# lRomul/sensorium

Hardware: AMD Instinct MI355X
Metric: training clips/sec/GPU (DwiseNeuro fwd+bwd, B=32 T=32 36x64) at 1/2/4/8 GPUs (higher is better)
Workload: dtype bf16

## Files before the change

include/dwn.h:

```cpp
#ifndef DWN_H_
#define DWN_H_
#include <stddef.h>
#include <stdint.h>

#ifdef __cplusplus
extern "C" {
#endif

#define DWN_ABI_VERSION 7
#define DWN_F32 0
#define DWN_BF16 1
#define DWN_F32_AUTO 0
#define DWN_F32_NATIVE 1
#define DWN_F32_SPLIT3 2
#define DWN_BN_EVAL 0
#define DWN_BN_TRAIN 1
#define DWN_BN_FROZEN 2
#define DWN_NREP 32

#define DWN_LD_PLAIN 0
#define DWN_LD_PE 1
#define DWN_LD_BNACT 2
#define DWN_LD_AFFINE2 3
#define DWN_LD_DY3 4
// ... 85 lines not shown
    void* dh1;
    float* dw;
    int planes, Hin, Win, Hout, Wout, C, stride, ks;
    double* stats;
    int rows_band;
    int impl;
    const void* a0; long long a0_ld; const void* w1; int Cin;
} dwn_dw_spatial_bwd_args;

typedef struct dwn_dw_temporal_fwd_args {
    dwn_load_desc in;
    const float* w;
    void* out;
    int B, T, HW, C, kt;
    double* stats;
    const float* z_scale; const float* z_shift; long long* pooled;
} dwn_dw_temporal_fwd_args;

typedef struct dwn_dw_temporal_bwd_args {
    dwn_load_desc dy; int dy_kind;
    dwn_load_desc y2;
    const float* w;
    void* dh2;
    float* dw;
    int B, T, HW, C, kt;
    double* stats;
} dwn_dw_temporal_bwd_args;

typedef struct dwn_bn {
    const float* gamma; const float* beta;
    float* running_mean; float* running_var; long long* num_batches_tracked;
    float* coef;
    float* dgamma; float* dbeta;
} dwn_bn;

typedef struct dwn_stem_args {
    int dtype, training, B, Cin, C0; long long S;
    float eps, momentum;
    const float* x;
    const float* w;
    dwn_bn bn;
    const float *pe_t, *pe_h, *pe_w;
    int T, H, W;
    void* y0;
    void* out;
    const void* dout;
    float* dw;
    void* ws; size_t ws_bytes;
    double* xmom;
} dwn_stem_args;

typedef struct dwn_stem_input_grad_args {
    int dtype, training, B, Cin, C0; long long S;
    const float* w;
    const float* coef;
    const void* dout;
    float* dx;
} dwn_stem_input_grad_args;

typedef struct dwn_block_args {
    int dtype, training;
    int B, T, Hin, Win, Hout, Wout, Cin, Cmid, Cout, stride, ks, kt, se_r;
    float eps, momentum;
    const void* x; void* out;
    void *y1, *y2, *y3, *y4;
    void* z3;
    int x_has_pe;
    void* a0;
    const float *pe_t, *pe_h, *pe_w;
    const float *out_pe_t, *out_pe_h, *out_pe_w;
    const float *w_pw, *w_dws, *w_dwt, *w_pwl, *se_wr, *se_br, *se_we, *se_be;
    dwn_bn bn1, bn2, bn3, bn4, bnsc;
    const float* drop_scale;
    const int *hsrc, *wsrc, *hinv, *winv;
    float *se_pmean, *se_hidpre, *se_gate;
    const void* dout; void* dx;
    void *buf_a, *buf_b;
    void *dy4, *da0;
    float *dw_pw, *dw_dws, *dw_dwt, *dw_pwl, *dse_wr, *dse_br, *dse_we, *dse_be;
    void* ws; size_t ws_bytes;
    int pwl_bwd;
    int f32_products;
    int y1_mode;
} dwn_block_args;

typedef struct dwn_pool_args {
    int dtype; long long BT; int HW, C;
    const void* x; void* out; const void* dout; void* dx;
} dwn_pool_args;

typedef struct dwn_cortex_args {
    int dtype, training, B, T, Cin, C, groups;
    float eps, momentum;
    const void* x; void* out; void* y;
    const float* w;
    dwn_bn bn, bnsc;
    const float* drop_scale;
    const void* dout; void* dx; float* dw;
    const float* dout_mask; int dout_mask_ld;
    void* ws; size_t ws_bytes;
    int f32_products;
} dwn_cortex_args;

typedef struct dwn_readout_args {
    int dtype, B, T, Cin, groups, n_out;
    float softplus_beta;
    const void* x;
    const float* w; const float* bias;
    const float* drop_mask;
    float* out;
    const float* dout; void* dx; float* dw; float* dbias;
    void* ws; size_t ws_bytes;
    void* wt;
    int f32_products;
    const float* beta_dev; float* dbeta;
} dwn_readout_args;

typedef struct dwn_tensor_entry {
    float* param; const float* grad; float* exp_avg; float* exp_avg_sq; float* ema;
    long long numel; int is_int64; int pad_;
} dwn_tensor_entry;

typedef struct dwn_guarded_entry {
    float* param; const float* grad; float* exp_avg; float* exp_avg_sq; float* ema;
    long long numel; int is_int64; int pad_;
    long long* step;
} dwn_guarded_entry;
typedef struct dwn_step_guard {
    double norm;
    float coef;
    int skip;
    long long nonfinite;
    long long good_steps, skipped_steps;
} dwn_step_guard;
#define DWN_GS_SEG 1024

#define DWN_VID_U8 0
#define DWN_VID_F32 1
typedef struct dwn_clip_src {
    const void* video; const float* behavior; const float* pupil_center; const float* responses;
    long long length;
    int video_dtype;
    int frame_start, frame_step;
    int valid;
} dwn_clip_src;
#define DWN_MIX_BOX 0
#define DWN_MIX_BLEND 1
typedef struct dwn_clip_desc {
    dwn_clip_src src, mix;
    int bbx1, bby1, bbx2, bby2;
    float one_minus_lam, lam;
    int mouse;
    int mix_mode;
} dwn_clip_desc;

enum {
    DWN_FAM_PW_FWD = 0, DWN_FAM_DWS_FWD, DWN_FAM_DWT_FWD, DWN_FAM_SE_POOL, DWN_FAM_PWL_FWD, DWN_FAM_RESID_FWD,
    DWN_FAM_RESID_BWD, DWN_FAM_PWL_DGRAD, DWN_FAM_PWL_WGRAD, DWN_FAM_BN3_REDUCE, DWN_FAM_DWT_BWD, DWN_FAM_DWS_BWD,
    DWN_FAM_PW_DGRAD, DWN_FAM_PW_WGRAD, DWN_FAM_CORTEX_FWD, DWN_FAM_CORTEX_BWD, DWN_FAM_READOUT_FWD, DWN_FAM_READOUT_BWD,
    DWN_FAM_COUNT
};
#define DWN_PROF_ROCTX (1ull << 63)
int dwn_profile_enable(unsigned long long family_mask, int device);
int dwn_profile_collect(int family, double* total_ms, long long* launches);

int dwn_abi_version(void);
const char* dwn_source_hash(void);
int dwn_sizeof(const char* struct_name);
const char* dwn_last_error(void);

int dwn_gemm_nn(const dwn_gemm_nn_args* a, int dtype, int device, void* stream);
int dwn_gemm_tn(const dwn_gemm_tn_args* a, int dtype, int device, void* stream);
int dwn_dw_spatial_fwd(const dwn_dw_spatial_fwd_args* a, int dtype, int device, void* stream);
int dwn_dw_spatial_bwd(const dwn_dw_spatial_bwd_args* a, int dtype, int device, void* stream);
int dwn_dw_spatial_fwd_rc_supported(const dwn_dw_spatial_fwd_args* a, int dtype);
int dwn_dw_spatial_bwd_rc_supported(const dwn_dw_spatial_bwd_args* a, int dtype);
int dwn_dw_temporal_fwd(const dwn_dw_temporal_fwd_args* a, int dtype, int device, void* stream);
int dwn_dw_temporal_bwd(const dwn_dw_temporal_bwd_args* a, int dtype, int device, void* stream);
int dwn_dw_temporal_wide_fwd(const dwn_dw_temporal_fwd_args* a, int dtype, int device, void* stream);
int dwn_dw_temporal_wide_bwd(const dwn_dw_temporal_bwd_args* a, int dtype, int device, void* stream);
int dwn_bn_finalize(const double* stats, int stat_c, double count, const dwn_bn* bn, int C, int training,
                    float momentum, float eps, int device, void* stream);
int dwn_bn_bwd_finalize(const double* stats, double count, const dwn_bn* bn, float* abc, int C, int device,
                        void* stream);
int dwn_pack_weight(const float* src, void* dst, int groups, int R, int C, int transpose, int Rd, int Cd,
                    int dtype, int device, void* stream);
size_t dwn_conv_pw_bn_stats_workspace_bytes(int Cin);
int dwn_conv_pw_bn_stats(const void* a0, long long a0_ld, long long M, const float* w_pw, int E, int Cin, const dwn_bn* bn,
                         float momentum, float eps, double* sc_stats, void* ws, size_t ws_bytes, int dtype, int device,
                         void* stream);

size_t dwn_stem_workspace_bytes(const dwn_stem_args* a);
int dwn_stem_forward(const dwn_stem_args* a, int device, void* stream);
int dwn_stem_backward(const dwn_stem_args* a, int device, void* stream);
int dwn_stem_input_grad(const dwn_stem_input_grad_args* a, int device, void* stream);
int dwn_stem_backward_input(const dwn_stem_args* a, float* dx, int device, void* stream);
size_t dwn_block_workspace_bytes(const dwn_block_args* a, int backward);
int dwn_block_forward(const dwn_block_args* a, int device, void* stream);
int dwn_block_backward(const dwn_block_args* a, int device, void* stream);
int dwn_block_forward_writes(const dwn_block_args* a);
int dwn_pool_forward(const dwn_pool_args* a, int device, void* stream);
int dwn_pool_backward(const dwn_pool_args* a, int device, void* stream);
size_t dwn_cortex_workspace_bytes(const dwn_cortex_args* a, int backward);
int dwn_cortex_forward(const dwn_cortex_args* a, int device, void* stream);
int dwn_cortex_backward(const dwn_cortex_args* a, int device, void* stream);
size_t dwn_readout_workspace_bytes(const dwn_readout_args* a, int backward);
size_t dwn_readout_wt_bytes(const dwn_readout_args* a);
int dwn_readout_forward(const dwn_readout_args* a, int device, void* stream);
int dwn_readout_backward(const dwn_readout_args* a, int device, void* stream);

int dwn_poisson_loss_forward(const float* pred, const float* target, const float* w, long long per_sample,
                             long long total, float eps, double* loss_acc, int device, void* stream);
int dwn_poisson_loss_backward(const float* pred, const float* target, const float* w, const float* gscale,
                              long long per_sample, long long total, float eps, float* dpred, int device,
                              void* stream);
int dwn_f64_to_f32(const double* src, float* dst, int n, int device, void* stream);

int dwn_adamw_ema_multi(const dwn_tensor_entry* list, int ntensors, int max_blocks, double lr, double beta1,
                        double beta2, double eps, double weight_decay, long long step, double ema_decay,
                        double grad_scale, int device, void* stream);
int dwn_ema_lerp_multi(const dwn_tensor_entry* list, int ntensors, int max_blocks, double decay, int device,
                       void* stream);

size_t dwn_grad_guard_workspace_bytes(int ntensors, int max_blocks);
int dwn_grad_sumsq_multi(const dwn_guarded_entry* list, int ntensors, int max_blocks, double grad_scale, void* ws,
                         size_t ws_bytes, double* pair, int device, void* stream);
int dwn_step_guard_finalize(const double* pair_a, const double* pair_b, double max_norm, int skip_nonfinite,
                            const dwn_guarded_entry* list, int ntensors, dwn_step_guard* guard, int device, void* stream);
int dwn_adamw_ema_multi_guarded(const dwn_guarded_entry* list, int ntensors, int max_blocks, double lr, double beta1,
                                double beta2, double eps, double weight_decay, double ema_decay, double grad_scale,
                                const dwn_step_guard* guard, int device, void* stream);


typedef struct dwn_pw_bwd_args {
    const void* dh1; const void* a0; const float* w_pw; const float* abc;
    void* da0; float* dw;
    long long M; int E; int Cin;
    void* ws; size_t ws_bytes;
    const void* res; const float* res_abc; int res_C;
    const int* res_hinv; const int* res_winv; int res_Hin, res_Win, res_Hout, res_Wout;
} dwn_pw_bwd_args;
int dwn_pw_bwd_fused_supported(int dtype, long long M, int E, int Cin);
size_t dwn_pw_backward_workspace_bytes(int E, int Cin, int dtype);
int dwn_pw_backward(const dwn_pw_bwd_args* a, int dtype, int device, void* stream);

typedef struct dwn_dw_spatial_rc_fwd_args {
    const void* a0; long long a0_ld;
    const void* blob;
    void* out;
    int planes, Hin, Win, Hout, Wout, Cin, E, stride;
    double* stats;
    int rows_band;
    int round_y1;
} dwn_dw_spatial_rc_fwd_args;
size_t dwn_dw_spatial_rc_blob_bytes(int E, int Cin);
int dwn_dw_spatial_rc_prep(const float* w_pw, const float* w_dws, const float* bn1_coef, int E, int Cin, void* blob,
                           int device, void* stream);
int dwn_dw_spatial_rc_supported(int dtype, int Cin, int E, int ks, int stride, int Hin, int Win);
int dwn_dw_spatial_fwd_rc(const dwn_dw_spatial_rc_fwd_args* a, int device, void* stream);

int dwn_assemble_inputs(const dwn_clip_desc* descs, int B, int T, int H0, int W0, int H, int W, float pad_fill,
                        float* x, int device, void* stream);
int dwn_assemble_targets(const dwn_clip_desc* descs, int B, int T, float* const* targets, const int* n_neurons,
                         int n_mice, int max_neurons, float* mice_weights, int device, void* stream);

typedef struct dwn_gaze_args {
    int B, Cin, T, H, W;
    int video_channel;
    float fill;
    int pad_;
    const float* x;
    const float* shift;
    float* out;
    const float* dout;
    float* dx;
    float* dshift;
} dwn_gaze_args;
int dwn_gaze_shift_forward(const dwn_gaze_args* a, int device, void* stream);
int dwn_gaze_shift_backward(const dwn_gaze_args* a, int device, void* stream);
int dwn_plane_mean(const float* x, int B, int Cin, int T, int H, int W, int c0, int nc, float* mean, int device, void* stream);

#define DWN_CORR_STAT_ROWS 8
#define DWN_CORR_TILE 16
// ... 208 lines not shown
```

sensorium_amd/_lib.py:

```python
from __future__ import annotations

import ctypes as C
import os
from pathlib import Path

import torch

_HERE = Path(__file__).resolve().parent
DETERMINISTIC = os.environ.get("DWN_DETERMINISTIC", "0") == "1"
_LIB_NAME = "libdwiseneuro_hip_det.so" if DETERMINISTIC else "libdwiseneuro_hip.so"
LIB_PATH = Path(os.environ["DWN_LIB_PATH"]) if os.environ.get("DWN_LIB_PATH") else _HERE / "csrc" / _LIB_NAME

c_p = C.c_void_p
c_i = C.c_int
c_ll = C.c_longlong
c_f = C.c_float
c_d = C.c_double
c_sz = C.c_size_t

DWN_F32, DWN_BF16 = 0, 1
DWN_NREP = 32
LD_PLAIN, LD_PE, LD_BNACT, LD_AFFINE2, LD_DY3, LD_GATE, LD_CAT1 = 0, 1, 2, 3, 4, 5, 6
EPI_STORE, EPI_READOUT, EPI_DG, EPI_STORE_CAT, EPI_DH3 = 0, 1, 2, 3, 4
NN_AUTO, NN_XL128, NN_XL256, NN_TILE128, NN_KD = 0, 1, 2, 3, 4
# ... 7 lines not shown
class LoadDesc(C.Structure):
    _fields_ = [("p", c_p), ("q", c_p), ("ld", c_ll), ("v1", c_p), ("v2", c_p), ("v3", c_p), ("v4", c_p),
                ("v5", c_p), ("gate", c_p), ("gate2", c_p), ("gate_ld", c_i), ("rows_per_sample", c_i),
                ("act", c_i), ("pe_t", c_p), ("pe_h", c_p), ("pe_w", c_p), ("pT", c_i), ("pH", c_i),
                ("pW", c_i), ("pe_ld", c_i), ("ld2", c_ll), ("cat_c1", c_i), ("cat_c2", c_i)]


class GemmNNArgs(C.Structure):
    _fields_ = [("a", LoadDesc), ("a_kind", c_i), ("b", c_p), ("ldb", c_ll), ("c", c_p), ("ldc", c_ll),
                ("M", c_i), ("N", c_i), ("K", c_i), ("groups", c_i), ("stats", c_p),
                ("f32_split", c_i), ("stat_nchan", c_i), ("epi", c_i), ("bias", c_p),
                ("sp_beta", c_f), ("out_nct", c_p), ("Tn", c_i), ("n_valid", c_i), ("y3", c_p), ("ldy3", c_ll),
                ("s3", c_p), ("t3", c_p), ("dg", c_p), ("dg_ld", c_i), ("rows_per_sample", c_i),
                ("a2", c_p), ("a2_ld", c_ll), ("K1", c_i), ("b_sample_stride", c_ll), ("b_rows_per_sample", c_i),
                ("gate3", c_p), ("dps3", c_p), ("coef3", c_p), ("coef3_ld", c_i), ("variant", c_i), ("sp_beta_dev", c_p)]


class GemmTNArgs(C.Structure):
    _fields_ = [("p", LoadDesc), ("p_kind", c_i), ("q", LoadDesc), ("q_kind", c_i), ("M", c_i), ("R", c_i),
                ("Cc", c_i), ("dw", c_p), ("lddw", c_ll), ("groups", c_i), ("rows_per_split", c_i),
                ("nsplit", c_i), ("R_load", c_i), ("rows_per_sample", c_i), ("splits_per_sample", c_i),
                ("dw_sample_stride", c_ll), ("overwrite", c_i), ("dw_f64", c_i)]


class DwSpatialFwdArgs(C.Structure):
    _fields_ = [("inp", LoadDesc), ("w", c_p), ("out", c_p), ("planes", c_i), ("Hin", c_i), ("Win", c_i),
                ("Hout", c_i), ("Wout", c_i), ("C", c_i), ("stride", c_i), ("ks", c_i), ("stats", c_p),
                ("rows_band", c_i), ("impl", c_i),
                ("a0", c_p), ("a0_ld", c_ll), ("w1", c_p), ("Cin", c_i)]


class DwSpatialBwdArgs(C.Structure):
    _fields_ = [("dy", LoadDesc), ("y1", LoadDesc), ("w", c_p), ("dh1", c_p), ("dw", c_p), ("planes", c_i),
                ("Hin", c_i), ("Win", c_i), ("Hout", c_i), ("Wout", c_i), ("C", c_i), ("stride", c_i),
                ("ks", c_i), ("stats", c_p), ("rows_band", c_i), ("impl", c_i),
                ("a0", c_p), ("a0_ld", c_ll), ("w1", c_p), ("Cin", c_i)]


class DwTemporalFwdArgs(C.Structure):
    _fields_ = [("inp", LoadDesc), ("w", c_p), ("out", c_p), ("B", c_i), ("T", c_i), ("HW", c_i), ("C", c_i),
                ("kt", c_i), ("stats", c_p), ("z_scale", c_p), ("z_shift", c_p), ("pooled", c_p)]


class DwTemporalBwdArgs(C.Structure):
    _fields_ = [("dy", LoadDesc), ("dy_kind", c_i), ("y2", LoadDesc), ("w", c_p), ("dh2", c_p), ("dw", c_p),
                ("B", c_i), ("T", c_i), ("HW", c_i), ("C", c_i), ("kt", c_i), ("stats", c_p)]


class BN(C.Structure):
    _fields_ = [("gamma", c_p), ("beta", c_p), ("running_mean", c_p), ("running_var", c_p),
                ("num_batches_tracked", c_p), ("coef", c_p), ("dgamma", c_p), ("dbeta", c_p)]


class StemArgs(C.Structure):
    _fields_ = [("dtype", c_i), ("training", c_i), ("B", c_i), ("Cin", c_i), ("C0", c_i), ("S", c_ll),
                ("eps", c_f), ("momentum", c_f), ("x", c_p), ("w", c_p), ("bn", BN),
                ("pe_t", c_p), ("pe_h", c_p), ("pe_w", c_p), ("T", c_i), ("H", c_i), ("W", c_i),
                ("y0", c_p), ("out", c_p),
                ("dout", c_p), ("dw", c_p), ("ws", c_p), ("ws_bytes", c_sz), ("xmom", c_p)]


class StemInputGradArgs(C.Structure):
    _fields_ = [("dtype", c_i), ("training", c_i), ("B", c_i), ("Cin", c_i), ("C0", c_i), ("S", c_ll),
                ("w", c_p), ("coef", c_p), ("dout", c_p), ("dx", c_p)]


class BlockArgs(C.Structure):
    _fields_ = [("dtype", c_i), ("training", c_i),
                ("B", c_i), ("T", c_i), ("Hin", c_i), ("Win", c_i), ("Hout", c_i), ("Wout", c_i), ("Cin", c_i),
                ("Cmid", c_i), ("Cout", c_i), ("stride", c_i), ("ks", c_i), ("kt", c_i), ("se_r", c_i),
                ("eps", c_f), ("momentum", c_f),
                ("x", c_p), ("out", c_p), ("y1", c_p), ("y2", c_p), ("y3", c_p), ("y4", c_p),
                ("z3", c_p), ("x_has_pe", c_i), ("a0", c_p),
                ("pe_t", c_p), ("pe_h", c_p), ("pe_w", c_p),
                ("out_pe_t", c_p), ("out_pe_h", c_p), ("out_pe_w", c_p),
                ("w_pw", c_p), ("w_dws", c_p), ("w_dwt", c_p), ("w_pwl", c_p), ("se_wr", c_p), ("se_br", c_p),
                ("se_we", c_p), ("se_be", c_p),
                ("bn1", BN), ("bn2", BN), ("bn3", BN), ("bn4", BN), ("bnsc", BN),
                ("drop_scale", c_p), ("hsrc", c_p), ("wsrc", c_p), ("hinv", c_p), ("winv", c_p),
                ("se_pmean", c_p), ("se_hidpre", c_p), ("se_gate", c_p),
                ("dout", c_p), ("dx", c_p), ("buf_a", c_p), ("buf_b", c_p), ("dy4", c_p), ("da0", c_p),
                ("dw_pw", c_p), ("dw_dws", c_p), ("dw_dwt", c_p), ("dw_pwl", c_p), ("dse_wr", c_p),
                ("dse_br", c_p), ("dse_we", c_p), ("dse_be", c_p),
                ("ws", c_p), ("ws_bytes", c_sz), ("pwl_bwd", c_i), ("f32_products", c_i), ("y1_mode", c_i)]


class PoolArgs(C.Structure):
    _fields_ = [("dtype", c_i), ("BT", c_ll), ("HW", c_i), ("C", c_i), ("x", c_p), ("out", c_p), ("dout", c_p),
                ("dx", c_p)]


class CortexArgs(C.Structure):
    _fields_ = [("dtype", c_i), ("training", c_i), ("B", c_i), ("T", c_i), ("Cin", c_i), ("C", c_i),
                ("groups", c_i), ("eps", c_f), ("momentum", c_f), ("x", c_p), ("out", c_p), ("y", c_p),
                ("w", c_p), ("bn", BN), ("bnsc", BN), ("drop_scale", c_p), ("dout", c_p), ("dx", c_p),
                ("dw", c_p), ("dout_mask", c_p), ("dout_mask_ld", c_i), ("ws", c_p), ("ws_bytes", c_sz), ("f32_products", c_i)]


class ReadoutArgs(C.Structure):
    _fields_ = [("dtype", c_i), ("B", c_i), ("T", c_i), ("Cin", c_i), ("groups", c_i), ("n_out", c_i),
                ("softplus_beta", c_f), ("x", c_p), ("w", c_p), ("bias", c_p), ("drop_mask", c_p), ("out", c_p),
                ("dout", c_p), ("dx", c_p), ("dw", c_p), ("dbias", c_p), ("ws", c_p), ("ws_bytes", c_sz), ("wt", c_p),
                ("f32_products", c_i), ("beta_dev", c_p), ("dbeta", c_p)]


class TensorEntry(C.Structure):
    _fields_ = [("param", c_p), ("grad", c_p), ("exp_avg", c_p), ("exp_avg_sq", c_p), ("ema", c_p),
                ("numel", c_ll), ("is_int64", c_i), ("pad_", c_i)]


class GuardedEntry(C.Structure):
    _fields_ = [("param", c_p), ("grad", c_p), ("exp_avg", c_p), ("exp_avg_sq", c_p), ("ema", c_p),
                ("numel", c_ll), ("is_int64", c_i), ("pad_", c_i), ("step", c_p)]


class StepGuard(C.Structure):
    _fields_ = [("norm", c_d), ("coef", c_f), ("skip", c_i), ("nonfinite", c_ll), ("good_steps", c_ll),
                ("skipped_steps", c_ll)]


class ClipSrc(C.Structure):
    _fields_ = [("video", c_p), ("behavior", c_p), ("pupil_center", c_p), ("responses", c_p), ("length", c_ll),
                ("video_dtype", c_i), ("frame_start", c_i), ("frame_step", c_i), ("valid", c_i)]


class ClipDesc(C.Structure):
    _fields_ = [("src", ClipSrc), ("mix", ClipSrc), ("bbx1", c_i), ("bby1", c_i), ("bbx2", c_i), ("bby2", c_i),
                ("one_minus_lam", c_f), ("lam", c_f), ("mouse", c_i), ("mix_mode", c_i)]


class PwBwdArgs(C.Structure):
    _fields_ = [("dh1", c_p), ("a0", c_p), ("w_pw", c_p), ("abc", c_p), ("da0", c_p), ("dw", c_p),
                ("M", c_ll), ("E", c_i), ("Cin", c_i), ("ws", c_p), ("ws_bytes", c_sz), ("res", c_p), ("res_abc", c_p),
                ("res_C", c_i), ("res_hinv", c_p), ("res_winv", c_p), ("res_Hin", c_i), ("res_Win", c_i), ("res_Hout", c_i),
                ("res_Wout", c_i)]


class DwSpatialRcFwdArgs(C.Structure):
    _fields_ = [("a0", c_p), ("a0_ld", c_ll), ("blob", c_p), ("out", c_p), ("planes", c_i), ("Hin", c_i),
                ("Win", c_i), ("Hout", c_i), ("Wout", c_i), ("Cin", c_i), ("E", c_i), ("stride", c_i),
                ("stats", c_p), ("rows_band", c_i), ("round_y1", c_i)]


class GazeArgs(C.Structure):
    _fields_ = [("B", c_i), ("Cin", c_i), ("T", c_i), ("H", c_i), ("W", c_i), ("video_channel", c_i), ("fill", c_f),
                ("pad_", c_i), ("x", c_p), ("shift", c_p), ("out", c_p), ("dout", c_p), ("dx", c_p), ("dshift", c_p)]


class CorrArgs(C.Structure):
    _fields_ = [("B", c_i), ("N", c_i), ("T", c_i), ("reduction", c_i), ("eps", c_d), ("w_stride", c_ll), ("pred", c_p),
                ("target", c_p), ("w", c_p), ("stat", c_p), ("count", c_p), ("share", c_p), ("loss_acc", c_p), ("gscale", c_p),
                ("dpred", c_p), ("ws", c_p), ("ws_bytes", c_sz)]


class GaborArgs(C.Structure):
    _fields_ = [("B", c_i), ("Cin", c_i), ("T", c_i), ("H", c_i), ("W", c_i), ("video_channel", c_i), ("envelope", c_i),
                ("clamp", c_i), ("y0", c_i), ("x0", c_i), ("wh", c_i), ("ww", c_i), ("background", c_f), ("lo", c_f), ("hi", c_f),
                ("pad", c_f), ("x", c_p), ("params", c_p), ("out", c_p), ("dout", c_p), ("dparams", c_p), ("ws", c_p),
                ("ws_bytes", c_sz)]


class ModulatorArgs(C.Structure):
    _fields_ = [("B", c_i), ("N", c_i), ("T", c_i), ("K", c_i), ("max_log_gain", c_f), ("pad_", c_i), ("y", c_p), ("h", c_p),
                ("u", c_p), ("c", c_p), ("out", c_p), ("dout", c_p), ("dy", c_p), ("dh", c_p), ("du", c_p), ("dc", c_p),
                ("ws", c_p), ("ws_bytes", c_sz)]


# ... 39 lines not shown
    _fields_ = [("B", c_i), ("Cin", c_i), ("T", c_i), ("H", c_i), ("W", c_i), ("video_channel", c_i), ("kind", c_i), ("cell", c_i),
                ("hold", c_i), ("y0", c_i), ("x0", c_i), ("wh", c_i), ("ww", c_i), ("pad_", c_i), ("background", c_f),
                ("contrast", c_f), ("density", c_f), ("pad", c_f), ("seed", C.c_ulonglong), ("first_clip", c_ll), ("x", c_p),
                ("out", c_p)]


class StaArgs(C.Structure):
    _fields_ = [("B", c_i), ("Cin", c_i), ("T", c_i), ("H", c_i), ("W", c_i), ("N", c_i), ("channel", c_i), ("y0", c_i), ("x0", c_i),
                ("wh", c_i), ("ww", c_i), ("cell", c_i), ("lags", c_i), ("skip", c_i), ("s0", c_f), ("pad_", c_i), ("samples", c_ll),
                ("rel_threshold", c_d), ("x", c_p), ("r", c_p), ("r0", c_p), ("state", c_p), ("cov", c_p), ("z", c_p),
                ("summary", c_p), ("ws", c_p), ("ws_bytes", c_sz)]


class Gauss2dArgs(C.Structure):
    _fields_ = [("R", c_i), ("gh", c_i), ("gw", c_i), ("M", c_i), ("fit_baseline", c_i), ("max_iter", c_i), ("rel_threshold", c_d),
                ("xtol", c_d), ("ftol", c_d), ("maps", c_p), ("sel", c_p), ("params", c_p), ("table", c_p), ("ws", c_p),
                ("ws_bytes", c_sz)]


class Gauss2dProfileArgs(C.Structure):
    _fields_ = [("N", c_i), ("L", c_i), ("gh", c_i), ("gw", c_i), ("fit_baseline", c_i), ("pad_", c_i), ("params", c_p), ("maps", c_p),
                ("profile", c_p), ("separability", c_p)]


CORR_STAT_ROWS, CORR_TILE = 8, 16
CORR_MEAN, CORR_SUM = 0, 1
GABOR_GAUSSIAN, GABOR_NONE = 0, 1
BLUR_MAX_RADIUS, BLUR_TAPS_STRIDE, MOMENTS_CHUNK = 16, 33, 4096
MEI_STEP, MEI_PROJECT = 0, 1
MEI_CONTRAST_MAX, MEI_CONTRAST_FIXED = 0, 1
TRIAL_STATE_ROWS, TRIAL_SCORE_ROWS, TRIAL_SUMMARY, TRIAL_TILE = 17, 5, 8, 4
NOISE_BINARY, NOISE_SPARSE = 0, 1
STA_SUMMARY = 8
GAUSS_PARAMS, GAUSS_TABLE = 7, 16
MIX_BOX, MIX_BLEND = 0, 1
VID_U8, VID_F32 = 0, 1

_STRUCTS = {
    "dwn_load_desc": LoadDesc, "dwn_gemm_nn_args": GemmNNArgs, "dwn_gemm_tn_args": GemmTNArgs,
    "dwn_dw_spatial_fwd_args": DwSpatialFwdArgs, "dwn_dw_spatial_bwd_args": DwSpatialBwdArgs,
    "dwn_dw_temporal_fwd_args": DwTemporalFwdArgs, "dwn_dw_temporal_bwd_args": DwTemporalBwdArgs,
    "dwn_bn": BN, "dwn_stem_args": StemArgs, "dwn_block_args": BlockArgs, "dwn_pool_args": PoolArgs,
    "dwn_cortex_args": CortexArgs, "dwn_readout_args": ReadoutArgs, "dwn_tensor_entry": TensorEntry,
    "dwn_clip_src": ClipSrc, "dwn_clip_desc": ClipDesc, "dwn_pw_bwd_args": PwBwdArgs,
    "dwn_dw_spatial_rc_fwd_args": DwSpatialRcFwdArgs, "dwn_stem_input_grad_args": StemInputGradArgs,
    "dwn_guarded_entry": GuardedEntry, "dwn_step_guard": StepGuard, "dwn_gaze_args": GazeArgs,
    "dwn_corr_args": CorrArgs, "dwn_gabor_args": GaborArgs, "dwn_modulator_args": ModulatorArgs,
    "dwn_blur3d_args": Blur3dArgs, "dwn_clip_moments_args": ClipMomentsArgs, "dwn_mei_update_args": MeiUpdateArgs,
    "dwn_trial_desc": TrialDesc, "dwn_trial_group": TrialGroup, "dwn_trial_score_args": TrialScoreArgs,
    "dwn_spatial_gain_args": SpatialGainArgs, "dwn_noise_args": NoiseArgs, "dwn_sta_args": StaArgs,
    "dwn_gauss2d_args": Gauss2dArgs, "dwn_gauss2d_profile_args": Gauss2dProfileArgs,
}

_P = C.POINTER
SYMBOLS = {
    "dwn_abi_version": (c_i, []),
    "dwn_source_hash": (C.c_char_p, []),
    "dwn_sizeof": (c_i, [C.c_char_p]),
    "dwn_last_error": (C.c_char_p, []),
    "dwn_profile_enable": (c_i, [C.c_ulonglong, c_i]),
    "dwn_profile_collect": (c_i, [c_i, _P(c_d), _P(c_ll)]),
    "dwn_gemm_nn": (c_i, [_P(GemmNNArgs), c_i, c_i, c_p]),
    "dwn_gemm_tn": (c_i, [_P(GemmTNArgs), c_i, c_i, c_p]),
    "dwn_dw_spatial_fwd": (c_i, [_P(DwSpatialFwdArgs), c_i, c_i, c_p]),
    "dwn_dw_spatial_bwd": (c_i, [_P(DwSpatialBwdArgs), c_i, c_i, c_p]),
    "dwn_dw_spatial_bwd_rc_supported": (c_i, [_P(DwSpatialBwdArgs), c_i]),
    "dwn_dw_spatial_fwd_rc_supported": (c_i, [_P(DwSpatialFwdArgs), c_i]),
    "dwn_dw_temporal_fwd": (c_i, [_P(DwTemporalFwdArgs), c_i, c_i, c_p]),
    "dwn_dw_temporal_bwd": (c_i, [_P(DwTemporalBwdArgs), c_i, c_i, c_p]),
    "dwn_dw_temporal_wide_fwd": (c_i, [_P(DwTemporalFwdArgs), c_i, c_i, c_p]),
    "dwn_dw_temporal_wide_bwd": (c_i, [_P(DwTemporalBwdArgs), c_i, c_i, c_p]),
    "dwn_bn_finalize": (c_i, [c_p, c_i, c_d, _P(BN), c_i, c_i, c_f, c_f, c_i, c_p]),
    "dwn_bn_bwd_finalize": (c_i, [c_p, c_d, _P(BN), c_p, c_i, c_i, c_p]),
    "dwn_pack_weight": (c_i, [c_p, c_p, c_i, c_i, c_i, c_i, c_i, c_i, c_i, c_i, c_p]),
    "dwn_stem_workspace_bytes": (c_sz, [_P(StemArgs)]),
    "dwn_stem_forward": (c_i, [_P(StemArgs), c_i, c_p]),
    "dwn_stem_backward": (c_i, [_P(StemArgs), c_i, c_p]),
    "dwn_stem_input_grad": (c_i, [_P(StemInputGradArgs), c_i, c_p]),
    "dwn_stem_backward_input": (c_i, [_P(StemArgs), c_p, c_i, c_p]),
    "dwn_block_workspace_bytes": (c_sz, [_P(BlockArgs), c_i]),
    "dwn_block_forward": (c_i, [_P(BlockArgs), c_i, c_p]),
    "dwn_block_backward": (c_i, [_P(BlockArgs), c_i, c_p]),
    "dwn_block_forward_writes": (c_i, [_P(BlockArgs)]),
    "dwn_pool_forward": (c_i, [_P(PoolArgs), c_i, c_p]),
    "dwn_pool_backward": (c_i, [_P(PoolArgs), c_i, c_p]),
    "dwn_cortex_workspace_bytes": (c_sz, [_P(CortexArgs), c_i]),
    "dwn_cortex_forward": (c_i, [_P(CortexArgs), c_i, c_p]),
    "dwn_cortex_backward": (c_i, [_P(CortexArgs), c_i, c_p]),
    "dwn_readout_workspace_bytes": (c_sz, [_P(ReadoutArgs), c_i]),
    "dwn_readout_wt_bytes": (c_sz, [_P(ReadoutArgs)]),
    "dwn_readout_forward": (c_i, [_P(ReadoutArgs), c_i, c_p]),
    "dwn_readout_backward": (c_i, [_P(ReadoutArgs), c_i, c_p]),
    "dwn_poisson_loss_forward": (c_i, [c_p, c_p, c_p, c_ll, c_ll, c_f, c_p, c_i, c_p]),
    "dwn_poisson_loss_backward": (c_i, [c_p, c_p, c_p, c_p, c_ll, c_ll, c_f, c_p, c_i, c_p]),
    "dwn_f64_to_f32": (c_i, [c_p, c_p, c_i, c_i, c_p]),
    "dwn_adamw_ema_multi": (c_i, [c_p, c_i, c_i, c_d, c_d, c_d, c_d, c_d, c_ll, c_d, c_d, c_i, c_p]),
    "dwn_ema_lerp_multi": (c_i, [c_p, c_i, c_i, c_d, c_i, c_p]),
    "dwn_grad_guard_workspace_bytes": (c_sz, [c_i, c_i]),
    "dwn_grad_sumsq_multi": (c_i, [c_p, c_i, c_i, c_d, c_p, c_sz, c_p, c_i, c_p]),
    "dwn_step_guard_finalize": (c_i, [c_p, c_p, c_d, c_i, c_p, c_i, c_p, c_i, c_p]),
    "dwn_adamw_ema_multi_guarded": (c_i, [c_p, c_i, c_i, c_d, c_d, c_d, c_d, c_d, c_d, c_d, c_p, c_i, c_p]),
    "dwn_conv_pw_bn_stats_workspace_bytes": (c_sz, [c_i]),
    "dwn_conv_pw_bn_stats": (c_i, [c_p, c_ll, c_ll, c_p, c_i, c_i, _P(BN), c_f, c_f, c_p, c_p, c_sz, c_i, c_i, c_p]),
    "dwn_pw_bwd_fused_supported": (c_i, [c_i, c_ll, c_i, c_i]),
    "dwn_pw_backward_workspace_bytes": (c_sz, [c_i, c_i, c_i]),
    "dwn_pw_backward": (c_i, [_P(PwBwdArgs), c_i, c_i, c_p]),
    "dwn_dw_spatial_rc_blob_bytes": (c_sz, [c_i, c_i]),
    "dwn_dw_spatial_rc_prep": (c_i, [c_p, c_p, c_p, c_i, c_i, c_p, c_i, c_p]),
    "dwn_dw_spatial_rc_supported": (c_i, [c_i, c_i, c_i, c_i, c_i, c_i, c_i]),
    "dwn_dw_spatial_fwd_rc": (c_i, [_P(DwSpatialRcFwdArgs), c_i, c_p]),
    "dwn_assemble_inputs": (c_i, [c_p, c_i, c_i, c_i, c_i, c_i, c_i, c_f, c_p, c_i, c_p]),
    "dwn_assemble_targets": (c_i, [c_p, c_i, c_i, c_p, c_p, c_i, c_i, c_p, c_i, c_p]),
    "dwn_gaze_shift_forward": (c_i, [_P(GazeArgs), c_i, c_p]),
    "dwn_gaze_shift_backward": (c_i, [_P(GazeArgs), c_i, c_p]),
    "dwn_plane_mean": (c_i, [c_p, c_i, c_i, c_i, c_i, c_i, c_i, c_i, c_p, c_i, c_p]),
    "dwn_corr_ws_bytes": (c_sz, [_P(CorrArgs)]),
    "dwn_corr_moments": (c_i, [_P(CorrArgs), c_i, c_p]),
    "dwn_corr_loss_finalize": (c_i, [_P(CorrArgs), c_i, c_p]),
    "dwn_corr_loss_backward": (c_i, [_P(CorrArgs), c_i, c_p]),
    "dwn_gabor_workspace_bytes": (c_sz, [_P(GaborArgs)]),
    "dwn_gabor_forward": (c_i, [_P(GaborArgs), c_i, c_p]),
    "dwn_gabor_backward": (c_i, [_P(GaborArgs), c_i, c_p]),
    "dwn_modulator_ws_bytes": (c_sz, [_P(ModulatorArgs)]),
    "dwn_modulator_forward": (c_i, [_P(ModulatorArgs), c_i, c_p]),
    "dwn_modulator_backward": (c_i, [_P(ModulatorArgs), c_i, c_p]),
    "dwn_blur3d_ws_bytes": (c_sz, [_P(Blur3dArgs)]),
    "dwn_clip_moments_ws_bytes": (c_sz, [_P(ClipMomentsArgs)]),
    "dwn_blur3d": (c_i, [_P(Blur3dArgs), c_i, c_p]),
    "dwn_clip_moments": (c_i, [_P(ClipMomentsArgs), c_i, c_p]),
    "dwn_mei_update": (c_i, [_P(MeiUpdateArgs), c_i, c_p]),
    "dwn_trial_score_ws_bytes": (c_sz, [_P(TrialScoreArgs)]),
    "dwn_trial_moments": (c_i, [_P(TrialScoreArgs), c_i, c_p]),
    "dwn_trial_score_finalize": (c_i, [_P(TrialScoreArgs), c_i, c_p]),
    "dwn_spatial_gain_ws_bytes": (c_sz, [_P(SpatialGainArgs)]),
    "dwn_spatial_gain_forward": (c_i, [_P(SpatialGainArgs), c_i, c_p]),
    "dwn_spatial_gain_backward": (c_i, [_P(SpatialGainArgs), c_i, c_p]),
    "dwn_gauss2d_ws_bytes": (c_sz, [_P(Gauss2dArgs)]),
    "dwn_gauss2d_fit": (c_i, [_P(Gauss2dArgs), c_i, c_p]),
    "dwn_gauss2d_profile": (c_i, [_P(Gauss2dProfileArgs), c_i, c_p]),
    "dwn_noise_forward": (c_i, [_P(NoiseArgs), c_i, c_p]),
    "dwn_sta_state_bytes": (c_sz, [_P(StaArgs)]),
    "dwn_sta_ws_bytes": (c_sz, [_P(StaArgs)]),
    "dwn_sta_accumulate": (c_i, [_P(StaArgs), c_i, c_p]),
    "dwn_sta_finalize": (c_i, [_P(StaArgs), c_i, c_p]),
}


class DwnError(RuntimeError):
    pass


HASH_SRCS = ("dwn_api.hip", "dwn_gemm.hip", "dwn_gemm_nn_1.hip", "dwn_gemm_nn_2.hip", "dwn_gemm_nn_3.hip", "dwn_gemm_nn_4.hip", "dwn_gemm_nn_5.hip",
             "dwn_gemm_nn_6.hip", "dwn_gemm_tn.hip", "dwn_pw_bwd.hip", "dwn_gemm_xl.hip", "dwn_gemm_kd.hip", "dwn_dwconv.hip", "dwn_dwrc.hip",
             "dwn_dwbwd.hip", "dwn_dwfwd.hip", "dwn_elementwise.hip", "dwn_data.hip", "dwn_gaze.hip", "dwn_modulator.hip", "dwn_spatial.hip", "dwn_mei.hip", "dwn_rf_fit.hip", "dwn_trial_score.hip", "dwn_rf.hip", "dwn_corr.hip", "dwn_stim.hip", "dwn_common.h", "dwn_internal.h",
             "dwn_kernels.h", "dwn_launch.h", "dwn_gemm_nn.h", "dwn_gain.h",
             "../../include/dwn.h")


def source_hash() -> str:
    import hashlib
    h = hashlib.sha256()
    for name in HASH_SRCS:
        h.update((_HERE / "csrc" / name).read_bytes())
    return h.hexdigest()[:16]


def _load():
    if not LIB_PATH.exists():
        raise ImportError(
            f"{LIB_PATH} is missing: build it with `python -c 'import __graft_entry__ as g; g.build()'` "
            f"(or `make -C {LIB_PATH.parent}`).  sensorium_amd has no fallback path.")
    lib = C.CDLL(str(LIB_PATH), mode=getattr(os, "RTLD_NOW", 2))
    ab = bool(os.environ.get("DWN_LIB_PATH"))
    for name, (restype, argtypes) in SYMBOLS.items():
        if ab and name in ("dwn_stem_input_grad", "dwn_stem_backward_input", "dwn_grad_guard_workspace_bytes", "dwn_grad_sumsq_multi",
                           "dwn_step_guard_finalize", "dwn_adamw_ema_multi_guarded", "dwn_dw_temporal_wide_fwd",
                           "dwn_dw_temporal_wide_bwd", "dwn_gaze_shift_forward", "dwn_gaze_shift_backward",
                           "dwn_plane_mean", "dwn_corr_ws_bytes", "dwn_corr_moments", "dwn_corr_loss_finalize",
                           "dwn_corr_loss_backward", "dwn_gabor_workspace_bytes", "dwn_gabor_forward",
                           "dwn_gabor_backward", "dwn_modulator_ws_bytes", "dwn_modulator_forward",
                           "dwn_modulator_backward", "dwn_blur3d_ws_bytes", "dwn_clip_moments_ws_bytes", "dwn_blur3d",
                           "dwn_clip_moments", "dwn_mei_update", "dwn_trial_score_ws_bytes", "dwn_trial_moments",
                           "dwn_trial_score_finalize", "dwn_spatial_gain_ws_bytes", "dwn_spatial_gain_forward",
                           "dwn_spatial_gain_backward", "dwn_noise_forward", "dwn_sta_state_bytes", "dwn_sta_ws_bytes",
                           "dwn_sta_accumulate", "dwn_sta_finalize", "dwn_gauss2d_ws_bytes", "dwn_gauss2d_fit",
                           "dwn_gauss2d_profile") and not hasattr(lib, name):
            continue
        fn = getattr(lib, name)
        fn.restype = restype
        fn.argtypes = argtypes
    if lib.dwn_abi_version() != 7 and not (ab and lib.dwn_abi_version() == 6):
        raise ImportError("libdwiseneuro_hip.so ABI version mismatch")
    built, have = lib.dwn_source_hash().decode(), source_hash()
    if built != have and not os.environ.get("DWN_LIB_PATH"):
        raise ImportError(f"{LIB_PATH.name} was built from other sources (binary {built}, tree {have}): rebuild it with "
                          f"`make -C {LIB_PATH.parent}` — binaries are not in git, so what runs must be what is committed")
    for cname, struct in _STRUCTS.items():
        n = lib.dwn_sizeof(cname.encode())
        if n != C.sizeof(struct) and not (ab and (0 < n < C.sizeof(struct) or cname in ("dwn_stem_input_grad_args", "dwn_guarded_entry", "dwn_step_guard", "dwn_gaze_args", "dwn_corr_args", "dwn_gabor_args", "dwn_modulator_args", "dwn_blur3d_args", "dwn_clip_moments_args", "dwn_mei_update_args", "dwn_trial_desc", "dwn_trial_group", "dwn_trial_score_args", "dwn_spatial_gain_args", "dwn_noise_args", "dwn_sta_args", "dwn_gauss2d_args", "dwn_gauss2d_profile_args"))):
            raise ImportError(f"struct layout mismatch for {cname}: C {n} bytes vs ctypes {C.sizeof(struct)}")
    return lib


lib = _load()


def check(rc: int, what: str = ""):
    if rc != 0:
        msg = lib.dwn_last_error()
        raise DwnError(f"{what} failed (rc={rc}): {msg.decode() if msg else ''}")
```

sensorium_amd/csrc/dwn_api.hip:

```cpp
#include "dwn_internal.h"
#include "dwn_kernels.h"
#include <string.h>
#include <math.h>

static thread_local char g_err[512] = "";
#ifndef DWN_EVAL_CHAIN
#define DWN_EVAL_CHAIN 1
#endif

extern "C" size_t dwn_dw_spatial_rc_blob_bytes(int E, int Cin);
extern "C" int dwn_dw_spatial_rc_supported(int dtype, int Cin, int E, int ks, int stride, int Hin, int Win);
extern "C" int dwn_dw_spatial_rc_prep(const float* w_pw, const float* w_dws, const float* bn1_coef, int E, int Cin, void* blob,
                                      int device, void* stream);
extern "C" int dwn_dw_spatial_fwd_rc(const dwn_dw_spatial_rc_fwd_args* a, int device, void* stream);
bool dw_spatial_bwd_rc_supported(const DwSpatialBwd& a, int dtype);
bool dw_spatial_fwd_rc_walk_supported(const DwSpatialFwd& a, int dtype);

int dwn_set_error(int code, const char* msg) {
    snprintf(g_err, sizeof(g_err), "dwn error %d: %s", code, msg ? msg : "");
    return code;
}

#define TRY(x) do { int rc__ = (x); if (rc__ != 0) return rc__; } while (0)

// ... 92 lines not shown
}
LoadDesc ld_ycoef(const void* y, i64 ld, const float* coef, int C) {
    LoadDesc d = ld_plain(y, ld);
    d.v1 = coef; d.v2 = coef + C; d.v3 = coef + 2 * C; d.v4 = coef + 3 * C;
    return d;
}

BnFinJob fin_job(const double* stats, int stat_c, double count, const dwn_bn& bn, int C) {
    BnFinJob j; memset(&j, 0, sizeof(j));
    j.stats = stats; j.stat_c = stat_c; j.count = count; j.gamma = bn.gamma; j.beta = bn.beta;
    j.running_mean = bn.running_mean; j.running_var = bn.running_var; j.nbt = bn.num_batches_tracked; j.coef = bn.coef; j.C = C;
    return j;
}
BnBwdJob bwd_job(const double* stats, double count, const dwn_bn& bn, float* abc, int C, bool frozen) {
    BnBwdJob j; memset(&j, 0, sizeof(j));
    j.stats = stats; j.count = count; j.coef = bn.coef; j.dgamma = bn.dgamma; j.dbeta = bn.dbeta; j.abc = abc; j.C = C;
    j.frozen = frozen ? 1 : 0;
    return j;
}

int bn_finalize(const double* stats, int stat_c, double count, const dwn_bn& bn, int C, int training, float momentum,
                float eps, hipStream_t s) {
    if (training) return k_bn_finalize_train(fin_job(stats, stat_c, count, bn, C), BnFinJob{}, momentum, eps, s);
    return k_bn_finalize_eval(bn.gamma, bn.beta, bn.running_mean, bn.running_var, eps, bn.coef, C, s);
}

GemmNN nn_base(const LoadDesc& a, int a_kind, const void* b, i64 ldb, void* c, i64 ldc, int M, int N, int K, int groups) {
    GemmNN g; memset(&g, 0, sizeof(g));
    g.a = a; g.a_kind = a_kind; g.b = b; g.ldb = ldb; g.c = c; g.ldc = ldc; g.M = M; g.N = N; g.K = K;
    g.groups = groups; g.epi = EPI_STORE;
    return g;
}
GemmTN tn_base(const LoadDesc& p, int pk, const LoadDesc& q, int qk, int M, int R, int Cc, float* dw, i64 lddw, int groups) {
    GemmTN g; memset(&g, 0, sizeof(g));
    g.p = p; g.p_kind = pk; g.q = q; g.q_kind = qk; g.M = M; g.R = R; g.Cc = Cc; g.dw = dw; g.lddw = lddw;
    g.groups = groups; g.nsplit = 0;
    return g;
}

struct BlockWs {
    void *wpw, *wpwl;
    float *wdws, *wdwt;
    double *st1, *st2, *st3, *st4, *stsc;
    long long* pooled;
    float *abc1, *abc2, *abc3, *abc4, *abcsc, *ident3;
    float *dgp, *dhp, *dps;
    void* bp; float* r3; float* gacc;
    float* tacc;
    void* wgated;
    void* rcblob;
    double* gram;
    float* pb;
    char* zero_beg; char* zero_end;
    size_t bytes;
};
#ifndef PWL_GATED_MIN_ROWS
#define PWL_GATED_MIN_ROWS 8192
#endif
static bool pwl_gated_weights(const dwn_block_args& a) {
    const int bk = a.dtype == DWN_BF16 ? 64 : 32;
    return ((a.T * a.Hout * a.Wout) % 128) == 0 && a.Cmid > bk && (a.dtype != DWN_BF16 || a.T * a.Hout * a.Wout >= PWL_GATED_MIN_ROWS);
}
static bool pwl_bwd_per_sample(const dwn_block_args& a) {
#ifdef DWN_DETERMINISTIC
    return true;
#endif
    if (a.pwl_bwd == 2) return false;
    if (a.pwl_bwd == 1) return true;
    const double pb = 4.0 * a.B * a.Cout * a.Cmid * sizeof(float);
    const double pass = (double)a.B * a.T * a.Hout * a.Wout * a.Cmid * tsize(a.dtype);
    return pb <= pass;
}
static bool block_y1_free(const dwn_block_args& a) {
    if (!a.training || a.dtype != DWN_BF16 || a.y1_mode == 1) return false;
    DwSpatialFwd f; memset(&f, 0, sizeof(f));
    f.planes = a.B * a.T; f.Hin = a.Hin; f.Win = a.Win; f.Hout = a.Hout; f.Wout = a.Wout; f.C = a.Cmid; f.stride = a.stride; f.ks = a.ks;
    f.in.ld = a.Cmid; f.a0_ld = a.Cin; f.Cin = a.Cin;
    if (!dw_spatial_fwd_rc_walk_supported(f, a.dtype)) return false;
    DwSpatialBwd d; memset(&d, 0, sizeof(d));
    d.planes = a.B * a.T; d.Hin = a.Hin; d.Win = a.Win; d.Hout = a.Hout; d.Wout = a.Wout; d.C = a.Cmid; d.stride = a.stride; d.ks = a.ks;
    d.dy.ld = a.Cmid; d.y1.ld = a.Cmid; d.a0_ld = a.Cin; d.Cin = a.Cin;
    if (!dw_spatial_bwd_rc_supported(d, a.dtype)) return false;
    return a.y1_mode == 2 || a.Cin == 64;
}
static bool block_fwd_rc(const dwn_block_args& a) {
    return !a.training && dwn_dw_spatial_rc_supported(a.dtype, a.Cin, a.Cmid, a.ks, a.stride, a.Hin, a.Win) != 0;
}
static size_t pw_fold_floats(int Cin) { return (size_t)Cin * Cin + Cin; }
BlockWs carve_block(const dwn_block_args& a, int backward, void* base, size_t cap) {
    BlockWs w; memset(&w, 0, sizeof(w));
    Carver c(base, cap);
    const size_t ts = tsize(a.dtype);
    w.wpw = c.take<char>((size_t)a.Cmid * a.Cin * ts);
    w.wpwl = c.take<char>((size_t)a.Cout * a.Cmid * ts);
    w.wdws = c.take<float>((size_t)a.ks * a.ks * a.Cmid);
    w.wdwt = c.take<float>((size_t)a.kt * a.Cmid);
    if (!backward && pwl_gated_weights(a)) w.wgated = c.take<char>((size_t)a.B * a.Cout * a.Cmid * ts);
    if (!backward && block_fwd_rc(a)) w.rcblob = c.take<char>(dwn_dw_spatial_rc_blob_bytes(a.Cmid, a.Cin));
    c.take<char>(0);
    size_t z0 = (c.off + 255) & ~(size_t)255;
    w.st1 = c.take<double>(nstat(a.Cmid));
    w.st2 = c.take<double>(nstat(a.Cmid));
    w.st3 = c.take<double>(nstat(a.Cmid));
    w.st4 = c.take<double>(nstat(a.Cout));
    w.stsc = c.take<double>(nstat(backward ? a.Cout : a.Cin));
    w.pooled = c.take<long long>((size_t)a.B * a.Cmid);
    if (!backward && block_y1_free(a)) w.gram = c.take<double>((size_t)(a.Cin + 8) * a.Cin);
    size_t z1 = c.off;
    if (backward) {
        w.abc1 = c.take<float>(3 * (size_t)a.Cmid);
        w.abc2 = c.take<float>(3 * (size_t)a.Cmid);
        w.abc3 = c.take<float>(3 * (size_t)a.Cmid);
        w.abc4 = c.take<float>(3 * (size_t)a.Cout);
        w.abcsc = c.take<float>(3 * (size_t)a.Cout);
        w.ident3 = c.take<float>(3 * (size_t)a.Cmid);
        w.dgp = c.take<float>((size_t)a.B * a.Cmid);
        w.dhp = c.take<float>((size_t)a.B * a.se_r);
        w.dps = c.take<float>((size_t)a.B * a.Cmid);
        w.bp = c.take<char>((size_t)a.Cin * (a.Cmid + a.Cin) * ts);
        w.gacc = c.take<float>(pw_fold_floats(a.Cin));
        w.r3 = w.gacc + (size_t)a.Cin * a.Cin;
        w.tacc = c.take<float>(pw_wgrad_tacc_floats(a.Cmid, a.Cin));
        if (pwl_bwd_per_sample(a)) w.pb = c.take<float>((size_t)a.B * a.Cout * a.Cmid);
    }
    w.bytes = c.off + 256;
    if (base) { w.zero_beg = (char*)base + z0; w.zero_end = (char*)base + z1; }
    return w;
}

static inline int f32_split_of(int policy, bool eval_forward) {
    return policy == DWN_F32_SPLIT3 ? 1 : policy == DWN_F32_NATIVE ? 0 : (eval_forward ? 1 : 0);
}

ResGeom geom_of(const dwn_block_args& a) {
    ResGeom gm;
    gm.BT = a.B * a.T; gm.T = a.T; gm.Hin = a.Hin; gm.Win = a.Win; gm.Hout = a.Hout; gm.Wout = a.Wout;
    gm.Cin = a.Cin; gm.Cout = a.Cout; gm.hsrc = a.hsrc; gm.wsrc = a.wsrc; gm.hinv = a.hinv; gm.winv = a.winv;
    return gm;
}

int check_block(const dwn_block_args& a) {
    if (a.Cin % 8 || a.Cmid % 8 || a.Cout % 8) return dwn_set_error(-2, "block: channel counts must be multiples of 8");
    if (a.ks != 3 && a.ks != 5 && a.ks != 7) return dwn_set_error(-4, "block: spatial_kernel must be 3, 5 or 7 (the built set)");
    if (a.kt != 3 && a.kt != 5 && a.kt != 7 && a.kt != 9) return dwn_set_error(-4, "block: temporal_kernel must be 3, 5, 7 or 9 (the built set)");
    if (a.Hout != (a.Hin - 1) / a.stride + 1 || a.Wout != (a.Win - 1) / a.stride + 1)
        return dwn_set_error(-2, "block: Hout/Wout inconsistent with stride");
    return 0;
}

}

extern "C" {

int dwn_abi_version(void) { return DWN_ABI_VERSION; }
int dwn_sizeof(const char* name) {
#define SZ(T) if (strcmp(name, #T) == 0) return (int)sizeof(T)
    SZ(dwn_load_desc); SZ(dwn_gemm_nn_args); SZ(dwn_gemm_tn_args); SZ(dwn_dw_spatial_fwd_args);
    SZ(dwn_dw_spatial_bwd_args); SZ(dwn_dw_temporal_fwd_args); SZ(dwn_dw_temporal_bwd_args); SZ(dwn_bn);
    SZ(dwn_stem_args); SZ(dwn_block_args); SZ(dwn_pool_args); SZ(dwn_cortex_args); SZ(dwn_readout_args);
    SZ(dwn_tensor_entry); SZ(dwn_clip_src); SZ(dwn_clip_desc); SZ(dwn_pw_bwd_args); SZ(dwn_dw_spatial_rc_fwd_args);
    SZ(dwn_stem_input_grad_args); SZ(dwn_guarded_entry); SZ(dwn_step_guard); SZ(dwn_gaze_args);
    SZ(dwn_corr_args); SZ(dwn_gabor_args); SZ(dwn_modulator_args); SZ(dwn_spatial_gain_args);
    SZ(dwn_blur3d_args); SZ(dwn_clip_moments_args); SZ(dwn_mei_update_args);
    SZ(dwn_trial_desc); SZ(dwn_trial_group); SZ(dwn_trial_score_args);
    SZ(dwn_noise_args); SZ(dwn_sta_args); SZ(dwn_gauss2d_args); SZ(dwn_gauss2d_profile_args);
#undef SZ
// ... 216 lines not shown
            ok = ok && pa.bneval(a.bn1, a.Cmid, a.eps) && pa.bneval(a.bn2, a.Cmid, a.eps) && pa.bneval(a.bn3, a.Cmid, a.eps);
            ok = ok && pa.bneval(a.bn4, a.Cout, a.eps) && pa.bneval(a.bnsc, a.Cout, a.eps);
        }
        if (!ok) return dwn_set_error(-2, "block_forward: workspace arena must be 16-byte aligned");
        TRY(k_prep(pa, dt, s));
    }

    const void* a0 = a.x;
    if (!a.x_has_pe) {
        if (!a.a0) return dwn_set_error(-2, "block_forward: a0 buffer required when x_has_pe == 0");
        TRY(k_ew_apply(ld_pe(a.x, a.Cin, a.pe_t, a.pe_h, a.pe_w, a.T, a.Hin, a.Win), LD_PE, a.a0, a.Cin, Min, a.Cin, dt, s));
        a0 = a.a0;
    }
    LoadDesc xin = ld_plain(a0, a.Cin);
    const bool identity_sc = a.stride == 1 && a.Hin == a.Hout && a.Win == a.Wout;
    const bool y1_free = tr && block_y1_free(a);
    bool eval_chain = false;
    if (DWN_EVAL_CHAIN && !tr && dt == DWN_BF16) {
        DwSpatialFwd f; memset(&f, 0, sizeof(f));
        f.planes = a.B * a.T; f.Hin = a.Hin; f.Win = a.Win; f.Hout = a.Hout; f.Wout = a.Wout; f.C = a.Cmid; f.stride = a.stride; f.ks = a.ks;
        f.in.ld = a.Cmid; f.a0_ld = a.Cin; f.Cin = a.Cin;
        eval_chain = dw_spatial_fwd_rc_walk_supported(f, dt);
    }
    if (eval_chain) {
        DwSpatialFwd d; memset(&d, 0, sizeof(d));
        d.in = ld_bnact(nullptr, a.Cmid, a.bn1.coef, a.Cmid, 1, nullptr, 0, 1);
        d.a0 = a0; d.a0_ld = a.Cin; d.w1 = w.wpw; d.Cin = a.Cin;
        d.w = w.wdws; d.out = a.y2; d.planes = a.B * a.T; d.Hin = a.Hin; d.Win = a.Win; d.Hout = a.Hout;
        d.Wout = a.Wout; d.C = a.Cmid; d.stride = a.stride; d.ks = a.ks; d.stats = nullptr;
        PROF(DWN_FAM_DWS_FWD, launch_dw_spatial_fwd(d, dt, s));
    } else if (y1_free) {
        LoadDesc cat = ld_plain(a0, a.Cin);
        cat.cat_c1 = a.Cin; cat.cat_c2 = 0;
        if (bs) {
        GemmTN g = tn_base(cat, LD_CAT1, ld_plain(a0, a.Cin), LD_PLAIN, (int)Min, a.Cin + 8, a.Cin, reinterpret_cast<float*>(w.gram), a.Cin, 1);
        g.dw_f64 = 1;
        PROF(DWN_FAM_PW_FWD, launch_gemm_tn(g, dt, s));
        PROF(DWN_FAM_PW_FWD, k_bn1_gram_finalize(w.gram, a.w_pw, a.Cmid, a.Cin, (double)Min, a.bn1.gamma, a.bn1.beta, a.bn1.running_mean,
                                                 a.bn1.running_var, a.bn1.num_batches_tracked, a.momentum, a.eps, a.bn1.coef,
                                                 identity_sc ? w.stsc : nullptr, dt, s));
        }
        DwSpatialFwd d; memset(&d, 0, sizeof(d));
        d.in = ld_bnact(nullptr, a.Cmid, a.bn1.coef, a.Cmid, 1, nullptr, 0, 1);
        d.a0 = a0; d.a0_ld = a.Cin; d.w1 = w.wpw; d.Cin = a.Cin;
        d.w = w.wdws; d.out = a.y2; d.planes = a.B * a.T; d.Hin = a.Hin; d.Win = a.Win; d.Hout = a.Hout;
        d.Wout = a.Wout; d.C = a.Cmid; d.stride = a.stride; d.ks = a.ks; d.stats = w.st2;
        PROF(DWN_FAM_DWS_FWD, launch_dw_spatial_fwd(d, dt, s));
    } else if (block_fwd_rc(a)) {
        TRY(dwn_dw_spatial_rc_prep(a.w_pw, w.wdws, a.bn1.coef, a.Cmid, a.Cin, w.rcblob, device, stream));
        dwn_dw_spatial_rc_fwd_args r; memset(&r, 0, sizeof(r));
        r.a0 = a0; r.a0_ld = a.Cin; r.blob = w.rcblob; r.out = a.y2; r.planes = a.B * a.T; r.Hin = a.Hin; r.Win = a.Win;
        r.Hout = a.Hout; r.Wout = a.Wout; r.Cin = a.Cin; r.E = a.Cmid; r.stride = a.stride; r.stats = nullptr;
        r.rows_band = 0; r.round_y1 = 1;
        PROF(DWN_FAM_DWS_FWD, dwn_dw_spatial_fwd_rc(&r, device, stream));
    } else {
    {
        GemmNN g = nn_base(xin, LD_PLAIN, w.wpw, a.Cin, a.y1, a.Cmid, (int)Min, a.Cmid, a.Cin, 1);
        g.f32_split = f32_split_of(a.f32_products, !tr);
        g.stats = tr ? w.st1 : nullptr; g.stat_nchan = a.Cmid;
        PROF(DWN_FAM_PW_FWD, launch_gemm_nn(g, dt, s));
    }
    if (bs) TRY(bn_finalize(w.st1, a.Cmid, (double)Min, a.bn1, a.Cmid, 1, a.momentum, a.eps, s));
    {
        DwSpatialFwd d; memset(&d, 0, sizeof(d));
        d.in = ld_bnact(a.y1, a.Cmid, a.bn1.coef, a.Cmid, 1, nullptr, 0, 1);
        d.w = w.wdws; d.out = a.y2; d.planes = a.B * a.T; d.Hin = a.Hin; d.Win = a.Win; d.Hout = a.Hout;
        d.Wout = a.Wout; d.C = a.Cmid; d.stride = a.stride; d.ks = a.ks; d.stats = tr ? w.st2 : nullptr;
        PROF(DWN_FAM_DWS_FWD, launch_dw_spatial_fwd(d, dt, s));
    }
    }
    if (bs) TRY(bn_finalize(w.st2, a.Cmid, (double)Mout, a.bn2, a.Cmid, 1, a.momentum, a.eps, s));
    const bool eval_z3 = !tr;
    {
        DwTemporalFwd d; memset(&d, 0, sizeof(d));
        d.in = ld_bnact(a.y2, a.Cmid, a.bn2.coef, a.Cmid, 1, nullptr, 0, 1);
        d.w = w.wdwt; d.out = a.y3; d.B = a.B; d.T = a.T; d.HW = a.Hout * a.Wout; d.C = a.Cmid; d.kt = a.kt;
        d.stats = tr ? w.st3 : nullptr;
        if (eval_z3) {
            d.out = a.z3; d.z_scale = a.bn3.coef; d.z_shift = a.bn3.coef + a.Cmid; d.pooled = w.pooled;
        }
        PROF(DWN_FAM_DWT_FWD, launch_dw_temporal_fwd(d, dt, s));
    }
    if (bs) TRY(bn_finalize(w.st3, a.Cmid, (double)Mout, a.bn3, a.Cmid, 1, a.momentum, a.eps, s));
    if (!eval_z3) {
        LoadDesc z3 = ld_bnact(a.y3, a.Cmid, a.bn3.coef, a.Cmid, 1, nullptr, 0, S_out);
        PROF(DWN_FAM_SE_POOL, k_se_pool(z3, a.B, a.Cmid, S_out, w.pooled, a.z3, dt, s));
    }
    int gate_folded = 0;
    TRY(k_se_mlp_fwd(w.pooled, 1.0f / (float)S_out, a.se_wr, a.se_br, a.se_we, a.se_be, a.B, a.Cmid, a.se_r,
                     a.se_pmean, a.se_hidpre, a.se_gate, pwl_gated_weights(a) ? a.w_pwl : nullptr, w.wgated, a.Cout, dt, &gate_folded, s));
    if (pwl_gated_weights(a)) {
        if (!gate_folded) TRY(k_gate_weights(a.w_pwl, a.se_gate, w.wgated, a.B, a.Cout, a.Cmid, dt, s));
        GemmNN g = nn_base(ld_plain(a.z3, a.Cmid), LD_PLAIN, w.wgated, a.Cmid, a.y4, a.Cout, (int)Mout, a.Cout, a.Cmid, 1);
        g.b_sample_stride = (i64)a.Cout * a.Cmid; g.b_rows_per_sample = S_out;
        g.stats = tr ? w.st4 : nullptr; g.stat_nchan = a.Cout; g.f32_split = f32_split_of(a.f32_products, !tr);
        PROF(DWN_FAM_PWL_FWD, launch_gemm_nn(g, dt, s));
    } else {
        LoadDesc u = ld_plain(a.z3, a.Cmid);
        u.gate = a.se_gate; u.gate_ld = a.Cmid; u.rows_per_sample = S_out;
        GemmNN g = nn_base(u, LD_GATE, w.wpwl, a.Cmid, a.y4, a.Cout, (int)Mout, a.Cout, a.Cmid, 1);
        g.stats = tr ? w.st4 : nullptr; g.stat_nchan = a.Cout; g.f32_split = f32_split_of(a.f32_products, !tr);
        PROF(DWN_FAM_PWL_FWD, launch_gemm_nn(g, dt, s));
    }
    ResGeom gm = geom_of(a);
    if (bs) {
        if (!(y1_free && identity_sc)) PROF(DWN_FAM_RESID_FWD, k_shortcut_stats(xin, gm, w.stsc, dt, s));
        TRY(k_bn_finalize_train(fin_job(w.st4, a.Cout, (double)Mout, a.bn4, a.Cout),
                                 fin_job(w.stsc, a.Cin, (double)Mout, a.bnsc, a.Cout), a.momentum, a.eps, s));
    }
    PROF(DWN_FAM_RESID_FWD, k_residual_fwd(xin, a.y4, a.bn4.coef, a.bnsc.coef, a.drop_scale, gm, a.out_pe_t, a.out_pe_h,
                                           a.out_pe_w, a.out, dt, s));
    return 0;
}

static int pw_backward(int dt, const void* dh1, const void* a0, const float* w_pw, const float* abc, int E, int Cin, i64 M,
                       void* bp, float* gacc, float* r3, float* tacc, void* da0, float* dw, const void* res,
                       const float* res_abc, int res_C, const ResGeom* rg, hipStream_t s) {
    const int res_n = res ? res_C / Cin : 0;
    const bool gathered = res && rg && rg->hinv;
    if (res && (!res_abc || res_C % Cin || res_n < 1 || res_n > 2))
        return dwn_set_error(-2, "pw_backward: the shortcut term needs res_abc and res_C in {Cin, 2 Cin}");
    if (res && !pw_bwd_fused_supported(dt, M, E, Cin))
        return dwn_set_error(-3, "pw_backward: the shortcut term is built into the one-pass kernel only (dwn_pw_bwd_fused_supported)");
    TRY(k_pw_bwd_prep(w_pw, abc, E, Cin, bp, gacc, r3, dt, (res && !gathered) ? res_abc : nullptr, res_C, s));
    if (pw_bwd_fused_supported(dt, M, E, Cin)) {
        PROF(DWN_FAM_PW_DGRAD, launch_pw_bwd_fused(dh1, a0, bp, r3, da0, tacc, M, E, Cin, dt, res, res_abc, res_n,
                                                   gathered ? rg->hinv : nullptr, gathered ? rg->winv : nullptr, gathered ? rg->Hin : 0,
                                                   gathered ? rg->Win : 0, gathered ? rg->Hout : 0, gathered ? rg->Wout : 0, s));
    } else {
        {
            GemmNN g = nn_base(ld_plain(dh1, E), LD_PLAIN, bp, (i64)E + Cin, da0, Cin, (int)M, Cin, E + Cin, 1);
            g.epi = EPI_STORE_CAT; g.a2 = a0; g.a2_ld = Cin; g.K1 = E; g.bias = r3;
            PROF(DWN_FAM_PW_DGRAD, launch_gemm_nn(g, dt, s));
        }
        {
            LoadDesc cat = ld_plain(dh1, E);
            cat.q = a0; cat.ld2 = Cin; cat.cat_c1 = E; cat.cat_c2 = Cin;
            GemmTN g = tn_base(cat, LD_CAT1, ld_plain(a0, Cin), LD_PLAIN, (int)M, E + Cin + 8, Cin, tacc, Cin, 1);
            PROF(DWN_FAM_PW_WGRAD, launch_gemm_tn(g, dt, s));
        }
    }
    return k_pw_wgrad_fold(tacc, abc, w_pw, E, Cin, dw, dt, s);
}

int dwn_block_backward(const dwn_block_args* ap, int device, void* stream) {
    const dwn_block_args& a = *ap;
    hipStream_t s = (hipStream_t)stream;
    g_err[0] = 0;
    TRY(check_block(a));
    if (a.training == DWN_BN_EVAL)
        return dwn_set_error(-7, "block_backward: only training-mode (batch-statistics) and frozen-statistics backward are built");
    ENTER(device);
    const bool frozen = a.training == DWN_BN_FROZEN;
    BlockWs w = carve_block(a, 1, a.ws, a.ws_bytes);
    if (w.bytes > a.ws_bytes) return dwn_set_error(-6, "block_backward: workspace too small");
    const int dt = a.dtype;
    const i64 Min = (i64)a.B * a.T * a.Hin * a.Win, Mout = (i64)a.B * a.T * a.Hout * a.Wout;
    const int S_out = a.T * a.Hout * a.Wout;
    float* dg = reinterpret_cast<float*>(w.pooled);
    const bool y1_free = block_y1_free(a);
    {
        PrepArgs pa;
        bool ok = pa.zero(w.zero_beg, ((size_t)(w.zero_end - w.zero_beg) + 15) & ~(size_t)15);
        ok = ok && pa.packw(a.w_pwl, w.wpwl, 1, a.Cout, a.Cmid, 1, a.Cmid, a.Cout);
        if (y1_free) ok = ok && pa.packw(a.w_pw, w.wpw, 1, a.Cmid, a.Cin, 0, a.Cmid, a.Cin);
        ok = ok && pa.packdw(a.w_dws, w.wdws, a.Cmid, a.ks * a.ks);
        ok = ok && pa.packdw(a.w_dwt, w.wdwt, a.Cmid, a.kt);
        ok = ok && pa.fill(w.ident3, 1.0f, a.Cmid);
        ok = ok && pa.fill(w.ident3 + a.Cmid, 0.0f, 2 * a.Cmid);
        ok = ok && pa.zero(a.dw_dws, (size_t)a.Cmid * a.ks * a.ks * sizeof(float));
        ok = ok && pa.zero(a.dw_dwt, (size_t)a.Cmid * a.kt * sizeof(float));
        ok = ok && pa.zero(a.dw_pwl, (size_t)a.Cout * a.Cmid * sizeof(float));
        if (w.pb) ok = ok && pa.zero(w.pb, (size_t)a.B * a.Cout * a.Cmid * sizeof(float));
        ok = ok && pa.zero(w.gacc, pw_fold_floats(a.Cin) * sizeof(float));
        ok = ok && pa.zero(w.tacc, pw_wgrad_tacc_floats(a.Cmid, a.Cin) * sizeof(float));
        if (!ok) return dwn_set_error(-2, "block_backward: workspace arena and dw_* buffers must be 16-byte aligned");
        TRY(k_prep(pa, dt, s));
    }

    LoadDesc xin = ld_plain(a.x_has_pe ? a.x : a.a0, a.Cin);
    ResGeom gm = geom_of(a);
    PROF(DWN_FAM_RESID_BWD, k_residual_bwd_reduce(xin, a.y4, a.dout, a.bn4.coef, a.bnsc.coef, a.drop_scale, gm, w.st4, w.stsc, dt, s));
    TRY(k_bn_bwd_finalize(bwd_job(w.st4, (double)Mout, a.bn4, w.abc4, a.Cout, frozen),
                          bwd_job(w.stsc, (double)Mout, a.bnsc, w.abcsc, a.Cout, frozen), s));
    PROF(DWN_FAM_RESID_BWD, k_residual_bwd_dy4(a.y4, a.dout, w.abc4, a.drop_scale, gm, a.dy4, dt, s));
    void* du = a.buf_a;
    if (w.pb) {
        {
            GemmTN g = tn_base(ld_plain(a.dy4, a.Cout), LD_PLAIN, ld_plain(a.z3, a.Cmid), LD_PLAIN, (int)Mout, a.Cout,
                               a.Cmid, w.pb, a.Cmid, 1);
            g.rows_per_sample = S_out; g.dw_sample_stride = (i64)a.Cout * a.Cmid;
            PROF(DWN_FAM_PWL_WGRAD, launch_gemm_tn(g, dt, s));
        }
        PROF(DWN_FAM_PWL_WGRAD, k_pwl_bwd_reduce(w.pb, a.se_gate, a.w_pwl, a.B, a.Cout, a.Cmid, a.dw_pwl, dg, s));
        TRY(k_se_mlp_bwd(dg, a.se_gate, a.se_hidpre, a.se_pmean, a.se_wr, a.se_we, a.B, a.Cmid, a.se_r,
                         1.0f / (float)S_out, w.dgp, w.dhp, w.dps, a.dse_wr, a.dse_br, a.dse_we, a.dse_be, s));
        GemmNN g = nn_base(ld_plain(a.dy4, a.Cout), LD_PLAIN, w.wpwl, a.Cout, du, a.Cmid, (int)Mout, a.Cmid, a.Cout, 1);
        g.epi = EPI_DH3; g.y3 = a.y3; g.ldy3 = a.Cmid; g.gate3 = a.se_gate; g.dps3 = w.dps; g.dg_ld = a.Cmid;
        g.coef3 = a.bn3.coef; g.coef3_ld = a.Cmid; g.rows_per_sample = S_out;
        g.stats = w.st3; g.stat_nchan = a.Cmid;
        PROF(DWN_FAM_PWL_DGRAD, launch_gemm_nn(g, dt, s));
    } else {
    {
        GemmNN g = nn_base(ld_plain(a.dy4, a.Cout), LD_PLAIN, w.wpwl, a.Cout, du, a.Cmid, (int)Mout, a.Cmid, a.Cout, 1);
        g.epi = EPI_DG; g.y3 = a.z3; g.ldy3 = a.Cmid; g.s3 = nullptr; g.t3 = nullptr; g.dg = dg;
        g.dg_ld = a.Cmid; g.rows_per_sample = S_out;
        PROF(DWN_FAM_PWL_DGRAD, launch_gemm_nn(g, dt, s));
    }
    {
        LoadDesc u = ld_plain(a.z3, a.Cmid);
        u.gate = a.se_gate; u.gate_ld = a.Cmid; u.rows_per_sample = S_out;
        GemmTN g = tn_base(ld_plain(a.dy4, a.Cout), LD_PLAIN, u, LD_GATE, (int)Mout, a.Cout, a.Cmid, a.dw_pwl, a.Cmid, 1);
        PROF(DWN_FAM_PWL_WGRAD, launch_gemm_tn(g, dt, s));
    }
    TRY(k_se_mlp_bwd(dg, a.se_gate, a.se_hidpre, a.se_pmean, a.se_wr, a.se_we, a.B, a.Cmid, a.se_r,
                     1.0f / (float)S_out, w.dgp, w.dhp, w.dps, a.dse_wr, a.dse_br, a.dse_we, a.dse_be, s));
    LoadDesc d3; memset(&d3, 0, sizeof(d3));
    d3.p = du; d3.q = a.y3; d3.ld = a.Cmid; d3.v1 = w.ident3; d3.v2 = w.ident3 + a.Cmid; d3.v3 = w.ident3 + 2 * a.Cmid;
    d3.v4 = a.bn3.coef; d3.v5 = a.bn3.coef + a.Cmid; d3.gate = a.se_gate; d3.gate2 = w.dps; d3.gate_ld = a.Cmid;
    d3.rows_per_sample = S_out;
    PROF(DWN_FAM_BN3_REDUCE, k_bn3_bwd_reduce(d3, a.bn3.coef, Mout, a.Cmid, w.st3, du, dt, s));
    }
    TRY(k_bn_bwd_finalize(bwd_job(w.st3, (double)Mout, a.bn3, w.abc3, a.Cmid, frozen), BnBwdJob{}, s));
    {
        DwTemporalBwd d; memset(&d, 0, sizeof(d));
        d.dy = ld_affine2(du, a.y3, a.Cmid, w.abc3, a.Cmid);
        d.dy_kind = LD_PLAIN;
        d.y2 = ld_ycoef(a.y2, a.Cmid, a.bn2.coef, a.Cmid);
        d.w = w.wdwt; d.dh2 = a.buf_b; d.dw = a.dw_dwt; d.B = a.B; d.T = a.T; d.HW = a.Hout * a.Wout; d.C = a.Cmid;
        d.kt = a.kt; d.stats = w.st2;
        PROF(DWN_FAM_DWT_BWD, launch_dw_temporal_bwd(d, dt, s));
    }
    TRY(k_bn_bwd_finalize(bwd_job(w.st2, (double)Mout, a.bn2, w.abc2, a.Cmid, frozen), BnBwdJob{}, s));
    void* dh1 = a.buf_a;
    {
        DwSpatialBwd d; memset(&d, 0, sizeof(d));
        d.dy = ld_affine2(a.buf_b, a.y2, a.Cmid, w.abc2, a.Cmid);
        d.y1 = ld_ycoef(y1_free ? nullptr : a.y1, a.Cmid, a.bn1.coef, a.Cmid);
        if (y1_free) { d.a0 = xin.p; d.a0_ld = a.Cin; d.w1 = w.wpw; d.Cin = a.Cin; }
        d.w = w.wdws; d.dh1 = dh1; d.dw = a.dw_dws; d.planes = a.B * a.T; d.Hin = a.Hin; d.Win = a.Win;
        d.Hout = a.Hout; d.Wout = a.Wout; d.C = a.Cmid; d.stride = a.stride; d.ks = a.ks; d.stats = w.st1;
        PROF(DWN_FAM_DWS_BWD, launch_dw_spatial_bwd(d, dt, s));
    }
    TRY(k_bn_bwd_finalize(bwd_job(w.st1, (double)Min, a.bn1, w.abc1, a.Cmid, frozen), BnBwdJob{}, s));
    const bool identity_sc = a.stride == 1 && a.Hin == a.Hout && a.Win == a.Wout;
    const bool dx_folded = a.Cout % a.Cin == 0 && a.Cout / a.Cin <= 2 && dwn_pw_bwd_fused_supported(dt, Min, a.Cmid, a.Cin) &&
                           (identity_sc || (gm.hinv && gm.winv && a.Hin + a.Win <= 512));
    TRY(pw_backward(dt, dh1, xin.p, a.w_pw, w.abc1, a.Cmid, a.Cin, Min, w.bp, w.gacc, w.r3, w.tacc, dx_folded ? a.dx : a.da0, a.dw_pw,
                    dx_folded ? a.dout : nullptr, w.abcsc, a.Cout, (dx_folded && !identity_sc) ? &gm : nullptr, s));
    if (dx_folded) return 0;
    PROF(DWN_FAM_RESID_BWD, k_residual_bwd_dx(xin, a.da0, a.dout, w.abcsc, gm, a.dx, dt, s));
    return 0;
}

int dwn_block_forward_writes(const dwn_block_args* ap) {
    const dwn_block_args& a = *ap;
    if (a.training) return block_y1_free(a) ? 2 : 3;
    if (block_fwd_rc(a)) return 0;
    if (DWN_EVAL_CHAIN && a.dtype == DWN_BF16) {
        DwSpatialFwd f; memset(&f, 0, sizeof(f));
        f.planes = a.B * a.T; f.Hin = a.Hin; f.Win = a.Win; f.Hout = a.Hout; f.Wout = a.Wout; f.C = a.Cmid; f.stride = a.stride; f.ks = a.ks;
        f.in.ld = a.Cmid; f.a0_ld = a.Cin; f.Cin = a.Cin;
        if (dw_spatial_fwd_rc_walk_supported(f, a.dtype)) return 0;
    }
    return 1;
}

int dwn_pool_forward(const dwn_pool_args* a, int device, void* stream) {
    ENTER(device);
    if (a->C % 8) return dwn_set_error(-2, "pool: C must be a multiple of 8");
    return k_pool_fwd(a->x, a->out, a->BT, a->HW, a->C, a->dtype, (hipStream_t)stream);
}
int dwn_pool_backward(const dwn_pool_args* a, int device, void* stream) {
    ENTER(device);
    if (a->C % 8) return dwn_set_error(-2, "pool: C must be a multiple of 8");
    return k_pool_bwd(a->dout, a->dx, a->BT, a->HW, a->C, a->dtype, (hipStream_t)stream);
}

namespace {
struct CortexWs { void* wp; double *st, *stsc; float *abc, *abcsc; void *dy, *dxmain; char *zb, *ze; size_t bytes; };
CortexWs carve_cortex(const dwn_cortex_args& a, int backward, void* base, size_t cap) {
    CortexWs w; memset(&w, 0, sizeof(w));
    Carver c(base, cap);
    const size_t ts = tsize(a.dtype);
    const i64 M = (i64)a.B * a.T;
    w.wp = c.take<char>((size_t)a.C * (a.Cin / a.groups) * ts);
    c.take<char>(0);
    size_t z0 = (c.off + 255) & ~(size_t)255;
    w.st = c.take<double>(nstat(a.C));
    w.stsc = c.take<double>(nstat(backward ? a.C : a.Cin));
    size_t z1 = c.off;
    if (backward) {
        w.abc = c.take<float>(3 * (size_t)a.C);
        w.abcsc = c.take<float>(3 * (size_t)a.C);
        w.dy = c.take<char>((size_t)M * a.C * ts);
        w.dxmain = c.take<char>((size_t)M * a.Cin * ts);
    }
    w.bytes = c.off + 256;
    if (base) { w.zb = (char*)base + z0; w.ze = (char*)base + z1; }
    return w;
}
}

size_t dwn_cortex_workspace_bytes(const dwn_cortex_args* a, int backward) {
    return carve_cortex(*a, backward, nullptr, 0).bytes;
}
int dwn_cortex_forward(const dwn_cortex_args* ap, int device, void* stream) {
    ENTER(device);
    const dwn_cortex_args& a = *ap;
    hipStream_t s = (hipStream_t)stream;
    if (a.Cin % (8 * a.groups) || a.C % (8 * a.groups)) return dwn_set_error(-2, "cortex: channels per group must be multiples of 8");
    CortexWs w = carve_cortex(a, 0, a.ws, a.ws_bytes);
    if (w.bytes > a.ws_bytes) return dwn_set_error(-6, "cortex_forward: workspace too small");
    const int M = a.B * a.T, Kg = a.Cin / a.groups, Ng = a.C / a.groups, dt = a.dtype, tr = a.training != DWN_BN_EVAL;
    const bool bs = a.training == DWN_BN_TRAIN;
    {
        PrepArgs pa;
        bool ok = pa.zero(w.zb, ((size_t)(w.ze - w.zb) + 15) & ~(size_t)15);
        ok = ok && pa.packw(a.w, w.wp, 1, a.C, Kg, 0, a.C, Kg);
        if (tr && !bs) ok = ok && pa.bneval(a.bn, a.C, a.eps) && pa.bneval(a.bnsc, a.C, a.eps);
        if (!ok) return dwn_set_error(-2, "cortex_forward: workspace arena must be 16-byte aligned");
        TRY(k_prep(pa, dt, s));
    }
    GemmNN g = nn_base(ld_plain(a.x, a.Cin), LD_PLAIN, w.wp, Kg, a.y, a.C, M, Ng, Kg, a.groups);
    g.f32_split = f32_split_of(a.f32_products, !tr);
    PROF(DWN_FAM_CORTEX_FWD, launch_gemm_nn(g, dt, s));
    if (bs) {
        TRY(k_cortex_stats(a.y, a.x, M, a.Cin, a.C, w.st, w.stsc, dt, s));
        TRY(k_bn_finalize_train(fin_job(w.st, a.C, (double)M, a.bn, a.C), fin_job(w.stsc, a.Cin, (double)M, a.bnsc, a.C),
                                 a.momentum, a.eps, s));
    } else if (!tr) {
        TRY(bn_finalize(w.st, a.C, (double)M, a.bn, a.C, 0, a.momentum, a.eps, s));
        TRY(bn_finalize(w.stsc, a.Cin, (double)M, a.bnsc, a.C, 0, a.momentum, a.eps, s));
    }
    return k_cortex_residual_fwd(a.y, a.x, a.bn.coef, a.bnsc.coef, a.drop_scale, M, a.T, a.Cin, a.C, a.groups, a.out,
                                 dt, s);
}
int dwn_cortex_backward(const dwn_cortex_args* ap, int device, void* stream) {
    const dwn_cortex_args& a = *ap;
    hipStream_t s = (hipStream_t)stream;
    g_err[0] = 0;
    if (a.training == DWN_BN_EVAL) return dwn_set_error(-7, "cortex_backward: only training-mode and frozen-statistics backward are built");
    ENTER(device);
    const bool frozen = a.training == DWN_BN_FROZEN;
    CortexWs w = carve_cortex(a, 1, a.ws, a.ws_bytes);
    if (w.bytes > a.ws_bytes) return dwn_set_error(-6, "cortex_backward: workspace too small");
    const int M = a.B * a.T, Kg = a.Cin / a.groups, Ng = a.C / a.groups, dt = a.dtype;
    {
        PrepArgs pa;
// ... 631 lines not shown
```

sensorium_amd/csrc/dwn_common.h:

```cpp
#pragma once
#include <hip/hip_runtime.h>
#include <stdint.h>
#include "../../include/dwn.h"

typedef uint16_t bf16_t;
typedef long long i64;


template <typename T> struct TT;
template <> struct TT<float>  { static constexpr int KC = 4; static constexpr int IS_BF16 = 0; };
template <> struct TT<bf16_t> { static constexpr int KC = 8; static constexpr int IS_BF16 = 1; };

__device__ __forceinline__ float bf2f(bf16_t v) { return __uint_as_float(((uint32_t)v) << 16); }
__device__ __forceinline__ bf16_t f2bf(float f) {
    __bf16 b = (__bf16)f;
    return __builtin_bit_cast(bf16_t, b);
}
typedef float dwn_f32x2_t __attribute__((ext_vector_type(2)));
typedef __bf16 dwn_bf16x2_t __attribute__((ext_vector_type(2)));
__device__ __forceinline__ uint32_t pk_bf16(float lo, float hi) {
    return __builtin_bit_cast(uint32_t, __builtin_convertvector(dwn_f32x2_t{lo, hi}, dwn_bf16x2_t));
}
template <typename T> __device__ __forceinline__ float to_f(T v);
template <> __device__ __forceinline__ float to_f<float>(float v) { return v; }
// ... 94 lines not shown
    return s * (1.0f + h * (1.0f - s));
}
template <int N> __device__ __forceinline__ void silu_n(float* v) {
    float s[N];
    sigmoid_n<N>(v, s);
#pragma unroll
    for (int i = 0; i < N; ++i) v[i] = v[i] * s[i];
}
template <int N> __device__ __forceinline__ void silu_grad_n(const float* h, float* g) {
    float s[N];
    sigmoid_n<N>(h, s);
#pragma unroll
    for (int i = 0; i < N; ++i) g[i] = s[i] * (1.0f + h[i] * (1.0f - s[i]));
}

template <typename T> struct V4 { };
template <> struct V4<float> {
    typedef uint4 raw_t;
    static constexpr int NCV = 8;
    static __device__ __forceinline__ void unpack(const raw_t& r, float* o) {
        o[0] = __uint_as_float(r.x); o[1] = __uint_as_float(r.y); o[2] = __uint_as_float(r.z); o[3] = __uint_as_float(r.w);
    }
    static __device__ __forceinline__ raw_t pack(const float* v) {
        return make_uint4(__float_as_uint(v[0]), __float_as_uint(v[1]), __float_as_uint(v[2]), __float_as_uint(v[3]));
    }
    static __device__ __forceinline__ raw_t zero() { return make_uint4(0, 0, 0, 0); }
};
template <> struct V4<bf16_t> {
    typedef uint2 raw_t;
    static constexpr int NCV = 16;
    static __device__ __forceinline__ void unpack(const raw_t& r, float* o) {
        o[0] = __uint_as_float(r.x << 16); o[1] = __uint_as_float(r.x & 0xffff0000u);
        o[2] = __uint_as_float(r.y << 16); o[3] = __uint_as_float(r.y & 0xffff0000u);
    }
    static __device__ __forceinline__ raw_t pack(const float* v) {
        uint2 r;
        r.x = pk_bf16(v[0], v[1]);
        r.y = pk_bf16(v[2], v[3]);
        return r;
    }
    static __device__ __forceinline__ raw_t zero() { return make_uint2(0, 0); }
};
template <typename T> __device__ __forceinline__ typename V4<T>::raw_t ld4_raw(const T* p) {
    return *reinterpret_cast<const typename V4<T>::raw_t*>(p);
}
template <typename T> __device__ __forceinline__ void ld4(const T* p, float* o) { V4<T>::unpack(ld4_raw<T>(p), o); }
template <typename T> __device__ __forceinline__ void st4(T* p, const float* v) {
    *reinterpret_cast<typename V4<T>::raw_t*>(p) = V4<T>::pack(v);
}
__device__ __forceinline__ void ldc4(const float* p, float* o) {
    float4 v = *reinterpret_cast<const float4*>(p);
    o[0] = v.x; o[1] = v.y; o[2] = v.z; o[3] = v.w;
}

enum { LD_PLAIN = 0, LD_PE = 1, LD_BNACT = 2, LD_AFFINE2 = 3, LD_DY3 = 4, LD_GATE = 5, LD_CAT1 = 6 };

typedef dwn_load_desc LoadDesc;

template <int KIND, typename T>
__device__ __forceinline__ void load_op(const LoadDesc& d, i64 row, int col, float* o) {
    constexpr int KC = TT<T>::KC;
    const T* p = reinterpret_cast<const T*>(d.p) + row * d.ld + col;
    ld_vec<T>(p, o);
    const unsigned r32 = (unsigned)row;
    if constexpr (KIND == LD_PE) {
        const unsigned r2 = r32 / (unsigned)d.pW;
        const int w = (int)(r32 - r2 * (unsigned)d.pW);
        const unsigned r3 = r2 / (unsigned)d.pH;
        const int h = (int)(r2 - r3 * (unsigned)d.pH);
        const int t = (int)(r3 % (unsigned)d.pT);
        float a[KC], b[KC], c[KC];
        ld_coef<KC>(d.pe_t + (i64)t * d.pe_ld + col, a);
        ld_coef<KC>(d.pe_h + (i64)h * d.pe_ld + col, b);
        ld_coef<KC>(d.pe_w + (i64)w * d.pe_ld + col, c);
#pragma unroll
        for (int i = 0; i < KC; ++i) o[i] = o[i] + ((a[i] + b[i]) + c[i]);
    } else if constexpr (KIND == LD_BNACT) {
        float s[KC], t[KC];
        ld_coef<KC>(d.v1 + col, s);
        ld_coef<KC>(d.v2 + col, t);
#pragma unroll
        for (int i = 0; i < KC; ++i) o[i] = fmaf(o[i], s[i], t[i]);
        if (d.act) silu_n<KC>(o);
        if (d.gate) {
            int b = (int)(r32 / (unsigned)d.rows_per_sample);
            float g[KC];
            ld_coef<KC>(d.gate + (i64)b * d.gate_ld + col, g);
#pragma unroll
            for (int i = 0; i < KC; ++i) o[i] *= g[i];
        }
    } else if constexpr (KIND == LD_GATE) {
        int b = (int)(r32 / (unsigned)d.rows_per_sample);
        float g[KC];
        ld_coef<KC>(d.gate + (i64)b * d.gate_ld + col, g);
#pragma unroll
        for (int i = 0; i < KC; ++i) o[i] *= g[i];
    } else if constexpr (KIND == LD_AFFINE2) {
        float y[KC], a1[KC], a2[KC], a3[KC];
        ld_vec<T>(reinterpret_cast<const T*>(d.q) + row * d.ld + col, y);
        ld_coef<KC>(d.v1 + col, a1);
        ld_coef<KC>(d.v2 + col, a2);
        ld_coef<KC>(d.v3 + col, a3);
#pragma unroll
        for (int i = 0; i < KC; ++i) o[i] = fmaf(a1[i], o[i], fmaf(a2[i], y[i], a3[i]));
    } else if constexpr (KIND == LD_DY3) {
        float y[KC], a1[KC], a2[KC], a3[KC], s[KC], t[KC], g[KC], g2[KC];
        ld_vec<T>(reinterpret_cast<const T*>(d.q) + row * d.ld + col, y);
        ld_coef<KC>(d.v1 + col, a1);
        ld_coef<KC>(d.v2 + col, a2);
        ld_coef<KC>(d.v3 + col, a3);
        ld_coef<KC>(d.v4 + col, s);
        ld_coef<KC>(d.v5 + col, t);
        int b = (int)(r32 / (unsigned)d.rows_per_sample);
        ld_coef<KC>(d.gate + (i64)b * d.gate_ld + col, g);
        ld_coef<KC>(d.gate2 + (i64)b * d.gate_ld + col, g2);
        float h[KC], sp[KC];
#pragma unroll
        for (int i = 0; i < KC; ++i) h[i] = fmaf(y[i], s[i], t[i]);
        silu_grad_n<KC>(h, sp);
#pragma unroll
        for (int i = 0; i < KC; ++i) {
            float dh = fmaf(o[i], g[i], g2[i]) * sp[i];
            o[i] = fmaf(a1[i], dh, fmaf(a2[i], y[i], a3[i]));
        }
    }
}

template <int KIND, typename T> struct ColCoef {
    static constexpr int KC = TT<T>::KC;
    float c1[KC], c2[KC], c3[KC], c4[KC], c5[KC], g[KC], g2[KC];
    int gb;
    int col;
    __device__ __forceinline__ void load(const LoadDesc& d, int column) {
        col = column; gb = -1;
        if constexpr (KIND == LD_BNACT) { ld_coef<KC>(d.v1 + col, c1); ld_coef<KC>(d.v2 + col, c2); }
        if constexpr (KIND == LD_AFFINE2 || KIND == LD_DY3) {
            ld_coef<KC>(d.v1 + col, c1); ld_coef<KC>(d.v2 + col, c2); ld_coef<KC>(d.v3 + col, c3);
        }
        if constexpr (KIND == LD_DY3) { ld_coef<KC>(d.v4 + col, c4); ld_coef<KC>(d.v5 + col, c5); }
    }
    __device__ __forceinline__ void gate_for(const LoadDesc& d, unsigned row) {
        int b = (int)(row / (unsigned)d.rows_per_sample);
        if (b != gb) {
            gb = b;
            ld_coef<KC>(d.gate + (i64)b * d.gate_ld + col, g);
            if constexpr (KIND == LD_DY3) ld_coef<KC>(d.gate2 + (i64)b * d.gate_ld + col, g2);
        }
    }
    __device__ __forceinline__ uint4 apply(const LoadDesc& d, unsigned row, const uint4& p, const uint4& q) {
        if constexpr (KIND == LD_PLAIN) { return p; }
        float o[KC];
        unpack16<T>(p, o);
        if constexpr (KIND == LD_GATE) {
            gate_for(d, row);
#pragma unroll
            for (int i = 0; i < KC; ++i) o[i] *= g[i];
        } else if constexpr (KIND == LD_BNACT) {
#pragma unroll
            for (int i = 0; i < KC; ++i) o[i] = fmaf(o[i], c1[i], c2[i]);
            if (d.act) silu_n<KC>(o);
            if (d.gate) {
                gate_for(d, row);
#pragma unroll
                for (int i = 0; i < KC; ++i) o[i] *= g[i];
            }
        } else if constexpr (KIND == LD_AFFINE2) {
            float y[KC];
            unpack16<T>(q, y);
#pragma unroll
            for (int i = 0; i < KC; ++i) o[i] = fmaf(c1[i], o[i], fmaf(c2[i], y[i], c3[i]));
        } else if constexpr (KIND == LD_DY3) {
            float y[KC];
            unpack16<T>(q, y);
            gate_for(d, row);
            float h[KC], sp[KC];
#pragma unroll
            for (int i = 0; i < KC; ++i) h[i] = fmaf(y[i], c4[i], c5[i]);
            silu_grad_n<KC>(h, sp);
#pragma unroll
            for (int i = 0; i < KC; ++i) {
                float dh = fmaf(o[i], g[i], g2[i]) * sp[i];
                o[i] = fmaf(c1[i], dh, fmaf(c2[i], y[i], c3[i]));
            }
        }
        return pack16<T>(o);
    }
    static constexpr bool two_tensors = (KIND == LD_AFFINE2 || KIND == LD_DY3);
};

#ifdef DWN_DETERMINISTIC
static __device__ unsigned dwn_det_ticket_ = 0;
__device__ __forceinline__ unsigned det_wg_id_() { return blockIdx.x + gridDim.x * (blockIdx.y + gridDim.y * blockIdx.z); }
__device__ __forceinline__ void det_enter_() {
    if (threadIdx.x == 0) {
        const unsigned me = det_wg_id_();
        while (__hip_atomic_load(&dwn_det_ticket_, __ATOMIC_ACQUIRE, __HIP_MEMORY_SCOPE_AGENT) != me) __builtin_amdgcn_s_sleep(16);
    }
    __syncthreads();
}
__device__ __forceinline__ void det_exit_() {
    det_enter_();
    if (threadIdx.x == 0) {
        __threadfence();
        unsigned next = det_wg_id_() + 1;
        if (next == gridDim.x * gridDim.y * gridDim.z) next = 0;
        __hip_atomic_store(&dwn_det_ticket_, next, __ATOMIC_RELEASE, __HIP_MEMORY_SCOPE_AGENT);
    }
}
#define DET_WAVES_BEGIN for (unsigned dw__ = 0; dw__ < (blockDim.x >> 6); ++dw__) { if ((threadIdx.x >> 6) == dw__) {
#define DET_WAVES_END } __syncthreads(); }
#define DET_ENTER() det_enter_()
#define DET_EXIT() det_exit_()
#define DET_ONLY(...) __VA_ARGS__
#else
#define DET_WAVES_BEGIN {
#define DET_WAVES_END }
#define DET_ENTER() ((void)0)
#define DET_EXIT() ((void)0)
#define DET_ONLY(...)
#endif

__device__ __forceinline__ void stat_add(double* base, int rep, int nchan, int which, int c, float v) {
    atomicAdd(base + ((i64)rep * 2 + which) * nchan + c, (double)v);
}

#define DWN_CHECK_LAUNCH() do { hipError_t e__ = hipGetLastError(); if (e__ != hipSuccess) return dwn_set_error((int)e__, hipGetErrorString(e__)); } while (0)

int dwn_set_error(int code, const char* msg);
```

sensorium_amd/csrc/dwn_elementwise.hip:

```cpp
#include "dwn_internal.h"
#include "dwn_kernels.h"
#include "dwn_launch.h"

#define NCV 8
#define DISPATCH_T(dtype, CALL_BF, CALL_F) do { if ((dtype) == DWN_BF16) { CALL_BF; } else { CALL_F; } } while (0)

#define SLICE_SETUP(Cval)                                   \
    constexpr int KC = TT<T>::KC;                           \
    const int tid = threadIdx.x;                            \
    const int cv = tid % NCV, pl = tid / NCV;               \
    const int c0 = blockIdx.y * NCV * KC;                   \
    const int chan = c0 + cv * KC;                          \
    const bool chan_ok = chan < (Cval);                     \
    (void)pl; (void)chan_ok;

template <int KC>
__device__ __forceinline__ void slice_stats_flush(float* lstat, const float* s0, const float* s1, int cv,
                                                 int c0, int C, double* stats, int rep) {
    static_assert(NCV == 8, "wave pre-reduction below assumes 8 channel vectors per slice");
    const int tid = threadIdx.x;
    DET_WAVES_BEGIN
#pragma unroll
    for (int i = 0; i < KC; ++i) {
        float a = s0[i], b = s1[i];
// ... 1014 lines not shown
        i64 routv[RES_RU];
#pragma unroll
        for (int u = 0; u < RES_RU; ++u) {
            const unsigned row = row0 + u * stride < rows ? row0 + u * stride : row0;
            unsigned bt; int hi, wi;
            ri.decode(row, bt, hi, wi);
            const int ho = ht_[hi], wo = wt_[wi];
            routv[u] = (ho >= 0 && wo >= 0) ? ((i64)bt * gm.Hout + ho) * gm.Wout + wo : -1;
            ra[u] = *reinterpret_cast<const uint4*>(da0 + (i64)row * gm.Cin + chan);
            rx[u] = make_uint4(0, 0, 0, 0);
            if (routv[u] >= 0) rx[u] = *reinterpret_cast<const uint4*>(xp + (i64)row * xin.ld + chan);
        }
#pragma unroll
        for (int u = 0; u < RES_RU; ++u) {
            const unsigned row = row0 + u * stride;
            if (row >= rows) break;
            float o[KC];
            unpack16<T>(ra[u], o);
            if (routv[u] >= 0) {
                float sv[KC];
                unpack16<T>(rx[u], sv);
                for (int cc = chan; cc < gm.Cout; cc += gm.Cin) {
                    float g[KC], a1[KC], a2[KC], a3[KC];
                    ld_vec<T>(dout + routv[u] * gm.Cout + cc, g);
                    ld_coef<KC>(abcsc + cc, a1); ld_coef<KC>(abcsc + gm.Cout + cc, a2);
                    ld_coef<KC>(abcsc + 2 * gm.Cout + cc, a3);
#pragma unroll
                    for (int i = 0; i < KC; ++i) o[i] += fmaf(a1[i], g[i], fmaf(a2[i], sv[i], a3[i]));
                }
            }
            st_vec<T>(dx + (i64)row * gm.Cin + chan, o);
        }
    }
}


int k_shortcut_stats(const LoadDesc& xin, const ResGeom& gm, double* stats, int dtype, hipStream_t s) {
    i64 rows = (i64)gm.BT * gm.Hout * gm.Wout;
    DISPATCH_T(dtype,
        hipLaunchKernelGGL((shortcut_stats_kernel<bf16_t>), fat_slice_grid(rows, gm.Cin, 8), dim3(STAT_NT), 0, s, xin, gm, stats),
        hipLaunchKernelGGL((shortcut_stats_kernel<float>), fat_slice_grid(rows, gm.Cin, 4), dim3(STAT_NT), 0, s, xin, gm, stats));
    DWN_CHECK_LAUNCH();
    return 0;
}
int k_residual_fwd(const LoadDesc& xin, const void* y4, const float* coef4, const float* coefsc, const float* dscale,
                   const ResGeom& gm, const float* ope_t, const float* ope_h, const float* ope_w, void* out, int dtype,
                   hipStream_t s) {
    i64 rows = (i64)gm.BT * gm.Hout * gm.Wout;
    DISPATCH_T(dtype,
        hipLaunchKernelGGL((residual_fwd_kernel<bf16_t>), slice_grid(rows, gm.Cout, 8), dim3(256), 0, s, xin, (const bf16_t*)y4, coef4, coefsc, dscale, gm, ope_t, ope_h, ope_w, (bf16_t*)out),
        hipLaunchKernelGGL((residual_fwd_kernel<float>), slice_grid(rows, gm.Cout, 4), dim3(256), 0, s, xin, (const float*)y4, coef4, coefsc, dscale, gm, ope_t, ope_h, ope_w, (float*)out));
    DWN_CHECK_LAUNCH();
    return 0;
}
int k_residual_bwd_reduce(const LoadDesc& xin, const void* y4, const void* dout, const float* coef4,
                          const float* coefsc, const float* dscale, const ResGeom& gm, double* stats4,
                          double* statssc, int dtype, hipStream_t s) {
    i64 rows = (i64)gm.BT * gm.Hout * gm.Wout;
    DISPATCH_T(dtype,
        hipLaunchKernelGGL((residual_bwd_reduce_kernel<bf16_t>), fat_slice_grid(rows, gm.Cout, 8), dim3(STAT_NT), 0, s, xin, (const bf16_t*)y4, (const bf16_t*)dout, coef4, coefsc, dscale, gm, stats4, statssc),
        hipLaunchKernelGGL((residual_bwd_reduce_kernel<float>), fat_slice_grid(rows, gm.Cout, 4), dim3(STAT_NT), 0, s, xin, (const float*)y4, (const float*)dout, coef4, coefsc, dscale, gm, stats4, statssc));
    DWN_CHECK_LAUNCH();
    return 0;
}
int k_residual_bwd_dy4(const void* y4, const void* dout, const float* abc4, const float* dscale, const ResGeom& gm,
                       void* dy4, int dtype, hipStream_t s) {
    i64 rows = (i64)gm.BT * gm.Hout * gm.Wout;
    DISPATCH_T(dtype,
        hipLaunchKernelGGL((residual_bwd_dy4_kernel<bf16_t>), slice_grid(rows, gm.Cout, 8), dim3(256), 0, s, (const bf16_t*)y4, (const bf16_t*)dout, abc4, dscale, gm, (bf16_t*)dy4),
        hipLaunchKernelGGL((residual_bwd_dy4_kernel<float>), slice_grid(rows, gm.Cout, 4), dim3(256), 0, s, (const float*)y4, (const float*)dout, abc4, dscale, gm, (float*)dy4));
    DWN_CHECK_LAUNCH();
    return 0;
}
int k_residual_bwd_dx(const LoadDesc& xin, const void* da0, const void* dout, const float* abcsc, const ResGeom& gm,
                      void* dx, int dtype, hipStream_t s) {
    i64 rows = (i64)gm.BT * gm.Hin * gm.Win;
    DISPATCH_T(dtype,
        hipLaunchKernelGGL((residual_bwd_dx_kernel<bf16_t>), slice_grid(rows, gm.Cin, 8), dim3(256), 0, s, xin, (const bf16_t*)da0, (const bf16_t*)dout, abcsc, gm, (bf16_t*)dx),
        hipLaunchKernelGGL((residual_bwd_dx_kernel<float>), slice_grid(rows, gm.Cin, 4), dim3(256), 0, s, xin, (const float*)da0, (const float*)dout, abcsc, gm, (float*)dx));
    DWN_CHECK_LAUNCH();
    return 0;
}

template <typename T>
__global__ __launch_bounds__(256) void se_pool_kernel(LoadDesc z3, int C, int rows_per_sample, int chunks,
                                                      long long* pooled, T* z3out) {
    SLICE_SETUP(C)
    __shared__ unsigned long long lacc[NCV * KC];
    if (tid < NCV * KC) lacc[tid] = 0ull;
    __syncthreads();
    const int b = blockIdx.x / chunks, chunk = blockIdx.x % chunks;
    const int per = (rows_per_sample + chunks - 1) / chunks;
    const int r_beg = chunk * per;
    const int r_end = (r_beg + per < rows_per_sample) ? r_beg + per : rows_per_sample;
    float acc[KC];
#pragma unroll
    for (int i = 0; i < KC; ++i) acc[i] = 0.f;
    if (chan_ok) {
        float sc[KC], sh[KC];
        ld_coef<KC>(z3.v1 + chan, sc);
        ld_coef<KC>(z3.v2 + chan, sh);
        const T* yp = reinterpret_cast<const T*>(z3.p);
        for (int r0 = r_beg + pl; r0 < r_end; r0 += 4 * 32) {
            uint4 raw[4];
#pragma unroll
            for (int u = 0; u < 4; ++u) {
                int r = r0 + 32 * u;
                raw[u] = *reinterpret_cast<const uint4*>(yp + ((i64)b * rows_per_sample + (r < r_end ? r : r_beg)) * z3.ld + chan);
            }
#pragma unroll
            for (int u = 0; u < 4; ++u) {
                int r = r0 + 32 * u;
                if (r >= r_end) break;
                float v[KC];
                unpack16<T>(raw[u], v);
#pragma unroll
                for (int i = 0; i < KC; ++i) v[i] = fmaf(v[i], sc[i], sh[i]);
                silu_n<KC>(v);
                if (z3out) st_vec<T>(z3out + ((i64)b * rows_per_sample + r) * C + chan, v);
#pragma unroll
                for (int i = 0; i < KC; ++i) acc[i] += round_t<T>(v[i]);
            }
        }
    }
#pragma unroll
    for (int i = 0; i < KC; ++i) atomicAdd(&lacc[cv * KC + i], (unsigned long long)pool_fix(acc[i]));
    __syncthreads();
    if (tid < NCV * KC && c0 + tid < C)
        atomicAdd(reinterpret_cast<unsigned long long*>(pooled) + (i64)b * C + c0 + tid, lacc[tid]);
}

int k_se_pool(const LoadDesc& z3, int B, int C, int rows_per_sample, long long* pooled, void* z3out, int dtype, hipStream_t s) {
    int KCv = dtype == DWN_BF16 ? 8 : 4;
    int slices = (C + NCV * KCv - 1) / (NCV * KCv);
    int chunks = (rows_per_sample + 255) / 256;
    int maxchunks = (2048 + B * slices - 1) / (B * slices);
    if (chunks > maxchunks) chunks = maxchunks;
    if (chunks < 1) chunks = 1;
    dim3 grid(B * chunks, slices);
    DISPATCH_T(dtype,
        hipLaunchKernelGGL((se_pool_kernel<bf16_t>), grid, dim3(256), 0, s, z3, C, rows_per_sample, chunks, pooled, (bf16_t*)z3out),
        hipLaunchKernelGGL((se_pool_kernel<float>), grid, dim3(256), 0, s, z3, C, rows_per_sample, chunks, pooled, (float*)z3out));
    DWN_CHECK_LAUNCH();
    return 0;
}

__global__ __launch_bounds__(256) void se_mlp_fwd_kernel(const long long* pooled_sum, float inv_s, const float* wr,
                                                         const float* br, const float* we, const float* be, int C,
                                                         int R, float* pmean, float* hid_pre, float* gate) {
    extern __shared__ float sh[];
    float* pm = sh;
    float* hid = sh + C;
    const int b = blockIdx.x, tid = threadIdx.x;
    const int split = gridDim.y, part = blockIdx.y;
    for (int c = tid; c < C; c += 256) {
        float v = pool_unfix(pooled_sum[(i64)b * C + c]) * inv_s;
        pm[c] = v;
        if (part == 0) pmean[(i64)b * C + c] = v;
    }
    __syncthreads();
    const int wave = tid >> 6, lane = tid & 63;
    for (int r = wave; r < R; r += 4) {
        float acc = 0.f;
        for (int c = lane; c < C; c += 64) acc = fmaf(wr[(i64)r * C + c], pm[c], acc);
        for (int o = 32; o > 0; o >>= 1) acc += __shfl_xor(acc, o);
        if (lane == 0) {
            float h = acc + br[r];
            if (part == 0) hid_pre[(i64)b * R + r] = h;
            hid[r] = siluf_(h);
        }
    }
    __syncthreads();
    const int per = (C + split - 1) / split;
    const int c_end = (part + 1) * per < C ? (part + 1) * per : C;
    for (int c = part * per + tid; c < c_end; c += 256) {
        float acc = be[c];
        for (int r = 0; r < R; ++r) acc = fmaf(we[(i64)c * R + r], hid[r], acc);
        gate[(i64)b * C + c] = sigmoidf_(acc);
    }
}

__global__ __launch_bounds__(256) void se_mlp_bwd_kernel(const float* dg, const float* gate, const float* hid_pre,
                                                         const float* wr, const float* we, int C, int R, float inv_s,
                                                         float* dgp_out, float* dhp_out, float* dps) {
    extern __shared__ float sh[];
    float* dgp = sh;
    float* dhp = sh + C;
    const int b = blockIdx.x, tid = threadIdx.x;
    const int split = gridDim.y, part = blockIdx.y;
    for (int c = tid; c < C; c += 256) {
        float g = gate[(i64)b * C + c];
        float v = dg[(i64)b * C + c] * g * (1.f - g);
        dgp[c] = v;
        if (part == 0) dgp_out[(i64)b * C + c] = v;
    }
    __syncthreads();
    const int wave = tid >> 6, lane = tid & 63;
    for (int r = wave; r < R; r += 4) {
        float acc = 0.f;
        for (int c = lane; c < C; c += 64) acc = fmaf(we[(i64)c * R + r], dgp[c], acc);
        for (int o = 32; o > 0; o >>= 1) acc += __shfl_xor(acc, o);
        if (lane == 0) {
            float v = acc * silu_gradf_(hid_pre[(i64)b * R + r]);
            dhp[r] = v;
            if (part == 0) dhp_out[(i64)b * R + r] = v;
        }
    }
    __syncthreads();
    const int per = (C + split - 1) / split;
    const int c_end = (part + 1) * per < C ? (part + 1) * per : C;
    for (int c = part * per + tid; c < c_end; c += 256) {
        float acc = 0.f;
        for (int r = 0; r < R; ++r) acc = fmaf(wr[(i64)r * C + c], dhp[r], acc);
        dps[(i64)b * C + c] = acc * inv_s;
    }
}

#define SE_RT 64
__device__ __forceinline__ float wave_sum(float v) {
#pragma unroll
    for (int o = 32; o > 0; o >>= 1) v += __shfl_xor(v, o);
    return v;
}

template <int RP>
// ... 1430 lines not shown
```

sensorium_amd/csrc/dwn_gemm_kd.hip:

```cpp
#include "dwn_internal.h"
#include "dwn_launch.h"
#include <type_traits>

#ifndef KD_FRG
#define KD_FRG 2
#endif
#ifndef KD_FRG256
#define KD_FRG256 1
#endif
#ifndef KD_WIDE
#define KD_WIDE 1
#endif
#ifndef KD_MINW128
#define KD_MINW128 3
#endif
typedef __attribute__((ext_vector_type(8))) short kd_bf16x8_t;
typedef __attribute__((ext_vector_type(4))) float kd_f32x4_t;

struct KdArgs {
    const bf16_t* A; i64 lda;
    const bf16_t* A2; i64 a2_ld; int K1;
    const bf16_t* B; i64 ldb;
    bf16_t* C; i64 ldc;
    int M, N, K;
    const float* bias;
    const float* gate; int gate_ld, rows_per_sample;
    double* stats; int stat_nchan;
    int ntm, ntn;
};

static __device__ __forceinline__ void kd_lds_barrier() {
    asm volatile("s_waitcnt lgkmcnt(0)" ::: "memory");
    __builtin_amdgcn_s_barrier();
    asm volatile("" ::: "memory");
}

template <int BN, int RT, bool GATE, bool CAT>
__global__ __launch_bounds__(256, BN * RT >= 512 ? 2 : KD_MINW128) void gemm_kd_kernel(const KdArgs g) {
    constexpr int BM = 64 * RT;
    constexpr int NJ = BN / 16;
    constexpr int NCH = BN * 4 / 256;
    constexpr int STG = BN * 64;
    constexpr int CROW = BN * 2 + 16;
    constexpr int CPR = BN / 8;
    constexpr int NIT = 64 * CPR / 256;
    constexpr int FRG = BN == 256 ? KD_FRG256 : KD_FRG;
    extern __shared__ __attribute__((aligned(16))) unsigned char kd_smem[];
    unsigned char* const sB = kd_smem;
    unsigned char* const sC = kd_smem + 2 * STG;
    float* const lred = reinterpret_cast<float*>(sC + 64 * CROW);
    float* const sgate = lred + 2 * BN;

    const int tid = threadIdx.x;
    const int wave = tid >> 6, lane = tid & 63, lr = lane & 15, lg = lane >> 4;
    const int t = (int)(blockIdx.x >> 3) + (int)(blockIdx.x & 7) * (int)(gridDim.x >> 3);
    const int nt = t % g.ntn, mt = t / g.ntn;
    if (mt >= g.ntm) { DET_EXIT(); return; }
    const int m0 = mt * BM, n0 = nt * BN;
    const int nk = g.K >> 5;

    const bf16_t* pa[RT];
    [[maybe_unused]] const bf16_t* pa2[RT];
#pragma unroll
    for (int i = 0; i < RT; ++i) {
        int m = m0 + 16 * RT * wave + 16 * i + lr;
        m = m < g.M ? m : g.M - 1;
        pa[i] = g.A + (i64)m * g.lda + 8 * lg;
        if constexpr (CAT) pa2[i] = g.A2 + (i64)m * g.a2_ld + 8 * lg;
    }
    uint4 ar[4][RT];
    auto load_a = [&](int ks, uint4 (&dst)[RT]) {
        ks = ks < nk ? ks : nk - 1;
        const int k = ks << 5;
#pragma unroll
        for (int i = 0; i < RT; ++i) {
            const bf16_t* src = pa[i] + k;
            if constexpr (CAT) src = k >= g.K1 ? pa2[i] + (k - g.K1) : src;
            dst[i] = *reinterpret_cast<const uint4*>(src);
        }
    };
    const bf16_t* pb[NCH];
    unsigned sboff[NCH];
#pragma unroll
    for (int i = 0; i < NCH; ++i) {
        const int c = tid + 256 * i, n = c >> 2, kc = c & 3;
        pb[i] = g.B + (i64)(n0 + n) * g.ldb + 8 * kc;
        sboff[i] = (unsigned)(n * 64 + ((kc ^ ((0 - (n >> 2)) & 3)) * 16));
    }
    uint4 bs[2][NCH];
    auto load_b = [&](int ks, uint4 (&dst)[NCH]) {
        ks = ks < nk ? ks : nk - 1;
#pragma unroll
        for (int i = 0; i < NCH; ++i) dst[i] = *reinterpret_cast<const uint4*>(pb[i] + (ks << 5));
    };
    auto store_b = [&](const int stage, const uint4 (&src)[NCH]) {
#pragma unroll
        for (int i = 0; i < NCH; ++i) *reinterpret_cast<uint4*>(sB + stage * STG + sboff[i]) = make_uint4(src[i].x, src[i].y, src[i].z, src[i].w);
    };

    kd_f32x4_t acc[RT][NJ];
#pragma unroll
    for (int i = 0; i < RT; ++i)
#pragma unroll
        for (int j = 0; j < NJ; ++j) acc[i][j] = kd_f32x4_t{0.f, 0.f, 0.f, 0.f};

#pragma unroll
    for (int u = 0; u < 4; ++u) load_a(u, ar[u]);
    load_b(0, bs[0]);
    load_b(1, bs[1]);
    if constexpr (GATE) {
        const float* grow = g.gate + (i64)(m0 / g.rows_per_sample) * g.gate_ld;
        for (int k = tid * 4; k < g.K; k += 1024) *reinterpret_cast<float4*>(sgate + k) = *reinterpret_cast<const float4*>(grow + k);
    }
    store_b(0, bs[0]);
    load_b(2, bs[0]);
    kd_lds_barrier();

    const unsigned char* const fb = sB + lr * 64 + ((lg ^ ((0 - (lr >> 2)) & 3)) * 16);
    auto step = [&](auto uc, const int ks) {
            constexpr int u = decltype(uc)::value;
            {
                constexpr int sb = (u + 1) & 1;
                const int kb = (ks + 3 < nk ? ks + 3 : nk - 1) << 5;
#pragma unroll
                for (int i = 0; i < NCH; ++i) {
                    *reinterpret_cast<uint4*>(sB + sb * STG + sboff[i]) = make_uint4(bs[sb][i].x, bs[sb][i].y, bs[sb][i].z, bs[sb][i].w);
                    bs[sb][i] = *reinterpret_cast<const uint4*>(pb[i] + kb);
                }
            }
            uint4 af[RT];
#pragma unroll
            for (int i = 0; i < RT; ++i) af[i] = ar[u][i];
            if constexpr (GATE) {
                const float4 g0 = *reinterpret_cast<const float4*>(sgate + (ks << 5) + 8 * lg);
                const float4 g1 = *reinterpret_cast<const float4*>(sgate + (ks << 5) + 8 * lg + 4);
                const float gv[8] = {g0.x, g0.y, g0.z, g0.w, g1.x, g1.y, g1.z, g1.w};
#pragma unroll
                for (int i = 0; i < RT; ++i) {
                    float v[8];
                    unpack16<bf16_t>(af[i], v);
#pragma unroll
                    for (int e = 0; e < 8; ++e) v[e] *= gv[e];
                    af[i] = pack16<bf16_t>(v);
                }
            }
            const unsigned char* const st = fb + (u & 1) * STG;
#pragma unroll
            for (int j0 = 0; j0 < NJ; j0 += FRG) {
                uint4 wf[FRG];
#pragma unroll
                for (int j = 0; j < FRG; ++j) wf[j] = *reinterpret_cast<const uint4*>(st + (j0 + j) * 1024);
                if constexpr (FRG > 1) __builtin_amdgcn_sched_barrier(0);
#pragma unroll
                for (int j = 0; j < FRG; ++j)
#pragma unroll
                    for (int i = 0; i < RT; ++i)
                        acc[i][j0 + j] = __builtin_amdgcn_mfma_f32_16x16x32_bf16(__builtin_bit_cast(kd_bf16x8_t, wf[j]), __builtin_bit_cast(kd_bf16x8_t, af[i]),
                                                                                 acc[i][j0 + j], 0, 0, 0);
            }
            if constexpr (u & 1) { load_a(ks + 3, ar[u - 1]); load_a(ks + 4, ar[u]); }
            kd_lds_barrier();
    };
    for (int ks0 = 0; ks0 < nk; ks0 += 4) {
        step(std::integral_constant<int, 0>{}, ks0);
        step(std::integral_constant<int, 1>{}, ks0 + 1);
        step(std::integral_constant<int, 2>{}, ks0 + 2);
        step(std::integral_constant<int, 3>{}, ks0 + 3);
    }

    const int ch = tid % CPR;
    float st0[8], st1[8];
#pragma unroll
    for (int e = 0; e < 8; ++e) { st0[e] = 0.f; st1[e] = 0.f; }
#pragma unroll
    for (int p = 0; p < BM / 64; ++p) {
        if (16 * RT * wave / 64 == p) {
#pragma unroll
            for (int i = 0; i < RT; ++i) {
                const int row = (16 * RT * wave) % 64 + 16 * i + lr;
#pragma unroll
                for (int j = 0; j < NJ; ++j) {
                    const int col = 16 * j + 4 * lg;
                    kd_f32x4_t v = acc[i][j];
                    if (g.bias) {
                        const float4 bv = *reinterpret_cast<const float4*>(g.bias + n0 + col);
                        v[0] += bv.x; v[1] += bv.y; v[2] += bv.z; v[3] += bv.w;
                    }
                    *reinterpret_cast<uint2*>(sC + row * CROW + col * 2) = make_uint2(pk_bf16(v[0], v[1]), pk_bf16(v[2], v[3]));
                }
            }
        }
        kd_lds_barrier();
#pragma unroll
        for (int it = 0; it < NIT; ++it) {
            const int row = tid / CPR + it * (256 / CPR);
            const int m = m0 + 64 * p + row;
            const uint4 raw = *reinterpret_cast<const uint4*>(sC + row * CROW + ch * 16);
            if (m < g.M) {
                *reinterpret_cast<uint4*>(g.C + (i64)m * g.ldc + n0 + ch * 8) = raw;
                float v[8];
                unpack16<bf16_t>(raw, v);
#pragma unroll
                for (int e = 0; e < 8; ++e) { st0[e] += v[e]; st1[e] = fmaf(v[e], v[e], st1[e]); }
            }
        }
        kd_lds_barrier();
    }
    if (g.stats) {
        for (int i = tid; i < 2 * BN; i += 256) lred[i] = 0.f;
        __syncthreads();
        DET_WAVES_BEGIN
#pragma unroll
        for (int e = 0; e < 8; ++e) {
            atomicAdd(&lred[ch * 8 + e], st0[e]);
            atomicAdd(&lred[BN + ch * 8 + e], st1[e]);
        }
        DET_WAVES_END
        __syncthreads();
        DET_ENTER();
        for (int i = tid; i < 2 * BN; i += 256)
            stat_add(g.stats, (int)(blockIdx.x % DWN_NREP), g.stat_nchan, i / BN, n0 + i % BN, lred[i]);
    }
    DET_EXIT();
}

static bool kd_args_ok(const GemmNN& g, int dtype) {
    if (dtype != DWN_BF16 || g.groups != 1 || g.b_sample_stride || g.M < 1) return false;
    if (g.epi == EPI_STORE) {
        if (g.a_kind != LD_PLAIN && g.a_kind != LD_GATE) return false;
        if (g.a2) return false;
    } else if (g.epi == EPI_STORE_CAT) {
        if (g.a_kind != LD_PLAIN || !g.a2 || !g.bias || g.K1 <= 0 || g.K1 % 32 || g.a2_ld % 8 || ((size_t)g.a2 & 15) || ((size_t)g.bias & 15)) return false;
    } else {
        return false;
    }
    if (g.a_kind == LD_GATE && (!g.a.gate || g.a.rows_per_sample <= 0 || g.a.rows_per_sample % 128 || g.a.gate_ld % 4 || ((size_t)g.a.gate & 15) || g.K > 4096))
        return false;
    if (g.K % 128 || g.N % 128 || g.a.ld % 8 || g.ldb % 8 || g.ldc % 8) return false;
    if (((size_t)g.a.p | (size_t)g.b | (size_t)g.c) & 15) return false;
    return true;
}

bool gemm_nn_kd_eligible(const GemmNN& g, int dtype) {
    if (g.variant == DWN_NN_TILE128 || g.variant == DWN_NN_XL128 || g.variant == DWN_NN_XL256) return false;
    if (!kd_args_ok(g, dtype)) return false;
    if (g.variant == DWN_NN_KD) return true;
    return g.K >= 512 && g.M >= 8192 && (g.N == 256 || (g.N == 128 && g.a_kind == LD_GATE));
}

template <int BN, int RT, bool GATE, bool CAT>
static int launch_kd_t(const KdArgs& a, hipStream_t s) {
    const size_t smem = 2 * (size_t)BN * 64 + 64 * ((size_t)BN * 2 + 16) + 2 * (size_t)BN * 4 + (GATE ? (size_t)a.K * 4 : 0);
    {
        hipError_t e = lds_opt_in(gemm_kd_kernel<BN, RT, GATE, CAT>, smem);
        if (e != hipSuccess) return dwn_set_error((int)e, hipGetErrorString(e));
    }
    const unsigned tiles = (unsigned)a.ntm * (unsigned)a.ntn;
    const unsigned grid = (tiles + 7u) & ~7u;
    hipLaunchKernelGGL((gemm_kd_kernel<BN, RT, GATE, CAT>), dim3(grid), dim3(256), smem, s, a);
    DWN_CHECK_LAUNCH();
    return 0;
}

int launch_gemm_nn_kd(const GemmNN& g, hipStream_t s) {
    KdArgs a;
    a.A = reinterpret_cast<const bf16_t*>(g.a.p); a.lda = g.a.ld;
    const bool cat = g.epi == EPI_STORE_CAT;
    a.A2 = cat ? reinterpret_cast<const bf16_t*>(g.a2) : nullptr; a.a2_ld = cat ? g.a2_ld : 0; a.K1 = cat ? g.K1 : g.K;
    a.B = reinterpret_cast<const bf16_t*>(g.b); a.ldb = g.ldb;
    a.C = reinterpret_cast<bf16_t*>(g.c); a.ldc = g.ldc;
    a.M = g.M; a.N = g.N; a.K = g.K;
    a.bias = cat ? g.bias : nullptr;
    const bool gate = g.a_kind == LD_GATE;
    a.gate = gate ? g.a.gate : nullptr; a.gate_ld = gate ? g.a.gate_ld : 0; a.rows_per_sample = gate ? g.a.rows_per_sample : 1;
    a.stats = g.stats; a.stat_nchan = g.stat_nchan;
    const int ntm128 = (g.M + 127) / 128;
    const bool wide = KD_WIDE && g.N % 256 == 0 && (i64)ntm128 * (g.N / 256) >= 512;
    a.ntm = ntm128;
    a.ntn = wide ? g.N / 256 : g.N / 128;
    if (wide) {
        if (gate) return launch_kd_t<256, 2, true, false>(a, s);
        return cat ? launch_kd_t<256, 2, false, true>(a, s) : launch_kd_t<256, 2, false, false>(a, s);
    }
    if (gate) return launch_kd_t<128, 2, true, false>(a, s);
    return cat ? launch_kd_t<128, 2, false, true>(a, s) : launch_kd_t<128, 2, false, false>(a, s);
}
```

sensorium_amd/csrc/dwn_gemm_tn.hip:

```cpp
#include "dwn_gemm_nn.h"
int k_zero(void* p, size_t nbytes, hipStream_t s);

#ifndef TN_MINW_PLAIN
#define TN_MINW_PLAIN 3
#endif
template <typename T> static __device__ __forceinline__ uint4 ones_vec();
template <> __device__ __forceinline__ uint4 ones_vec<bf16_t>() { return make_uint4(0x3F803F80u, 0x3F803F80u, 0x3F803F80u, 0x3F803F80u); }
template <> __device__ __forceinline__ uint4 ones_vec<float>() { return make_uint4(0x3F800000u, 0x3F800000u, 0x3F800000u, 0x3F800000u); }
template <typename T> struct TnCfg;
template <> struct TnCfg<bf16_t> { static constexpr int PAD = 32; };
template <> struct TnCfg<float>  { static constexpr int PAD = 64; };

template <int PLD, int QLD> struct TnOcc {
    static constexpr int value = (PLD == LD_AFFINE2 || PLD == LD_DY3 || QLD == LD_AFFINE2 || QLD == LD_DY3) ? 2 : TN_MINW_PLAIN;
};
template <typename T, int PLD, int QLD>
__global__ __launch_bounds__(256, (TnOcc<PLD, QLD>::value)) void gemm_tn_kernel(const GemmTN g) {
    constexpr int KC = TT<T>::KC;
    constexpr int BR = 128, BC = 128, BMK = TT<T>::IS_BF16 ? 64 : 32;
    constexpr int RS = BR * (int)sizeof(T) + TnCfg<T>::PAD;
    constexpr int CPR = BR / KC;
    constexpr int NCH = BMK * CPR / 256;
    __shared__ __attribute__((aligned(16))) unsigned char smem[2 * BMK * RS];
    unsigned char* sP = smem;
    unsigned char* sQ = smem + BMK * RS;

    const int tid = threadIdx.x;
    const int ntc = (g.Cc + BC - 1) / BC;
    int tile_id = blockIdx.x, split_id = blockIdx.y;
    {
        const unsigned total = gridDim.x * gridDim.y, bid = blockIdx.x + gridDim.x * blockIdx.y;
        if ((total & 7u) == 0u) {
            const unsigned lid = (bid & 7u) * (total >> 3) + (bid >> 3);
            tile_id = (int)(lid % gridDim.x);
            split_id = (int)(lid / gridDim.x);
        }
    }
    const int rt = tile_id / ntc, ct = tile_id % ntc;
    const int r0 = rt * BR, c0 = ct * BC;
    const int grp = blockIdx.z;
    const int Rl = g.R_load > 0 ? g.R_load : g.R;
    const int pcol0 = grp * Rl, qcol0 = grp * g.Cc;
    i64 mbeg = (i64)split_id * g.rows_per_split;
    i64 mend = mbeg + g.rows_per_split;
    if (mend > g.M) mend = g.M;
    i64 dw_off = 0;
    if (g.rows_per_sample > 0) {
        const int b = split_id / g.splits_per_sample, j = split_id % g.splits_per_sample;
        mbeg = (i64)b * g.rows_per_sample + (i64)j * g.rows_per_split;
        mend = mbeg + g.rows_per_split;
        const i64 send = (i64)(b + 1) * g.rows_per_sample;
        if (mend > send) mend = send;
        dw_off = (i64)b * g.dw_sample_stride;
    }

    const int wave = tid >> 6, lane = tid & 63;
    const int wm = wave >> 1, wn = wave & 1;
    const int lr = lane & 15, lg = lane >> 4;

    f32x4_t acc[4][4];
#pragma unroll
    for (int i = 0; i < 4; ++i)
#pragma unroll
        for (int j = 0; j < 4; ++j) acc[i][j] = f32x4_t{0.f, 0.f, 0.f, 0.f};

    uint4 p1[NCH], p2[NCH], q1[NCH], q2[NCH];
    i64 ld_mb = 0;
    const int chq = tid % CPR;
    const int rcol = r0 + chq * KC, ccol = c0 + chq * KC;
    const bool rok = rcol < Rl, cok = ccol < g.Cc;
    ColCoef<(PLD == LD_PE || PLD == LD_CAT1) ? LD_PLAIN : PLD, T> cfp;
    ColCoef<QLD == LD_PE ? LD_PLAIN : QLD, T> cfq;
    if (rok) cfp.load(g.p, pcol0 + rcol);
    if (cok) cfq.load(g.q, qcol0 + ccol);
    const T* Pp = reinterpret_cast<const T*>(g.p.p);
    const T* Pq = reinterpret_cast<const T*>(g.p.q);
    const T* Qp = reinterpret_cast<const T*>(g.q.p);
    const T* Qq = reinterpret_cast<const T*>(g.q.q);
    i64 pld = g.p.ld;
    int pcol = pcol0 + rcol;
    [[maybe_unused]] bool p_ones = false;
    if constexpr (PLD == LD_CAT1) {
        if (rcol >= g.p.cat_c1 + g.p.cat_c2) p_ones = true;
        else if (rcol >= g.p.cat_c1) { Pp = Pq; pld = g.p.ld2; pcol = rcol - g.p.cat_c1; }
    }
    auto load_tiles = [&](i64 mb) {
        ld_mb = mb;
#pragma unroll
        for (int i = 0; i < NCH; ++i) {
            i64 m = mb + tid / CPR + (256 / CPR) * i;
            const bool mok = m < mend;
            i64 offp = (mok && rok) ? m * pld + pcol : 0;
            if constexpr (PLD == LD_CAT1) { if (p_ones) offp = 0; }
            const i64 offq = (mok && cok) ? m * g.q.ld + qcol0 + ccol : 0;
            if constexpr (PLD != LD_PE) {
                p1[i] = *reinterpret_cast<const uint4*>(Pp + offp);
                if constexpr (decltype(cfp)::two_tensors) p2[i] = *reinterpret_cast<const uint4*>(Pq + offp);
// ... 202 lines not shown
```

sensorium_amd/ops.py:

```python
from __future__ import annotations

import ctypes as C
import math
import os
import threading
from typing import Optional

import numpy as np
import torch
from torch.autograd.function import once_differentiable

from . import _lib as L

_DT = {torch.float32: L.DWN_F32, torch.bfloat16: L.DWN_BF16}


def _ptr(t: Optional[torch.Tensor]):
    return None if t is None else t.data_ptr()


def _stream(device: torch.device):
    return torch.cuda.current_stream(device).cuda_stream


# ... 3 lines not shown
                           "the HIP path has no CPU fallback")


def _bn_struct(bn: torch.nn.modules.batchnorm._BatchNorm, coef: torch.Tensor, dgamma=None, dbeta=None) -> L.BN:
    s = L.BN()
    s.gamma = bn.weight.data_ptr()
    s.beta = bn.bias.data_ptr()
    s.running_mean = bn.running_mean.data_ptr()
    s.running_var = bn.running_var.data_ptr()
    s.num_batches_tracked = bn.num_batches_tracked.data_ptr()
    s.coef = coef.data_ptr()
    s.dgamma = _ptr(dgamma)
    s.dbeta = _ptr(dbeta)
    return s


def _check_bn(bn):
    if bn.momentum is None or not bn.affine or not bn.track_running_stats:
        raise RuntimeError("sensorium_amd: BatchNorm must be affine with running stats and a fixed momentum")


def _f32_products(mod, inference_readout: bool = False) -> int:
    native = getattr(mod, "_dwn_fp32_native", False)
    if inference_readout:
        return L.F32_NATIVE if native else L.F32_SPLIT3
    return L.F32_NATIVE if native else L.F32_AUTO


_EVAL_BACKWARD_ERROR = "sensorium_amd: backward through eval-mode BatchNorm is not built"


class _BnModeState(threading.local):
    override: Optional[int] = None


_BN_MODE = _BnModeState()


class bn_mode_scope:

    def __init__(self, mode: Optional[int]):
        self.mode = mode

    def __enter__(self):
        self.prev, _BN_MODE.override = _BN_MODE.override, self.mode
        return self

    def __exit__(self, *exc):
        _BN_MODE.override = self.prev
        return False


def wants_frozen(x: torch.Tensor, switch: bool = False) -> bool:
    return torch.is_grad_enabled() and (bool(x.requires_grad) or switch)


def bn_mode(training: bool, x: torch.Tensor) -> int:
    if training:
        return L.BN_TRAIN
    if _BN_MODE.override is not None:
        return _BN_MODE.override
    return L.BN_FROZEN if wants_frozen(x) else L.BN_EVAL


def _ddp_flush() -> None:
    from . import ddp
    if ddp._LIVE:
        ddp.flush_ready_all()


def _ws(nbytes: int, device) -> torch.Tensor:
    return torch.empty(int(nbytes), dtype=torch.uint8, device=device)


def _env_choice(name: str, table: dict) -> int:
    v = os.environ.get(name, "")
    if v not in table:
        raise ValueError(f"{name}={v!r}: expected one of {sorted(k for k in table if k)} (or unset)")
    return table[v]


_PWL_BWD = _env_choice("DWN_PWL_BWD", {"": 0, "new": 1, "old": 2})
_Y1_MODE = _env_choice("DWN_Y1", {"": 0, "free": 0, "materialise": 1, "all": 2})


def grad_out(param: torch.Tensor, zero: bool = False) -> torch.Tensor:
    slot = getattr(param, "_dwn_grad_slot", None)
    if slot is not None and param.grad is None and not getattr(param, "_dwn_slot_out", False):
        param._dwn_slot_out = True
        flat, off = slot
        g = flat[off:off + param.numel()].view(param.shape)
        return g.zero_() if zero else g
    if zero:
        return torch.zeros_like(param, dtype=torch.float32)
    return torch.empty_like(param, dtype=torch.float32)


def nearest_src_index(out_size: int, in_size: int) -> np.ndarray:
    scale = np.float32(in_size) / np.float32(out_size)
    src = np.floor(np.arange(out_size, dtype=np.float32) * scale).astype(np.int64)
    return np.minimum(src, in_size - 1).astype(np.int32)


def inverse_index(src: np.ndarray, in_size: int) -> np.ndarray:
    inv = np.full(in_size, -1, dtype=np.int32)
    inv[src] = np.arange(len(src), dtype=np.int32)
    if len(np.unique(src)) != len(src):
        raise RuntimeError("nearest-neighbour shortcut map is not injective (stride < 1?)")
    return inv


def pe_axis_tables(channels: int, inv_freq: torch.Tensor, t: int, h: int, w: int):
    ch = int(math.ceil(channels / 6) * 2)
    if ch % 2:
        ch += 1
    inv = inv_freq.detach().float().cpu()
    tabs = []
    for axis, size in enumerate((t, h, w)):
        arg = inv[:, None] * torch.arange(size).float()[None, :]
        emb = torch.cat([arg.sin(), arg.cos()], dim=0)
        tab = torch.zeros(size, channels, dtype=torch.float32)
        lo = axis * ch
        n = max(0, min(ch, channels - lo))
        if n > 0:
            tab[:, lo:lo + n] = emb[:n].t()
        tabs.append(tab.contiguous())
    return tabs


class StemFn(torch.autograd.Function):

    @staticmethod
    def forward(ctx, x, weight, gamma, beta, mod, dtype, pe=None, mode=None):
        _require_gpu(x, "StemFn")
        conv, bn = mod.stem[0], mod.stem[1].bn
        _check_bn(bn)
        if mode is None:
            mode = int(bn.training)
        x = x.contiguous().float()
        B, Cin, T, H, W = x.shape
        C0 = weight.shape[0]
        dev = x.device
        out = torch.empty(B, T, H, W, C0, dtype=dtype, device=dev)
        coef = torch.empty(4 * C0, dtype=torch.float32, device=dev)
        xmom = torch.empty(72, dtype=torch.float64, device=dev)
        a = L.StemArgs()
        a.dtype = _DT[dtype]; a.training = mode; a.B = B; a.Cin = Cin; a.C0 = C0; a.S = T * H * W
        a.eps = bn.eps; a.momentum = bn.momentum
        a.x = x.data_ptr(); a.w = weight.data_ptr(); a.bn = _bn_struct(bn, coef)
        a.out = out.data_ptr(); a.xmom = xmom.data_ptr()
        if pe is not None:
            a.pe_t, a.pe_h, a.pe_w = (t.data_ptr() for t in pe)
        a.T, a.H, a.W = T, H, W
        ws = _ws(L.lib.dwn_stem_workspace_bytes(C.byref(a)), dev)
        a.ws = ws.data_ptr(); a.ws_bytes = ws.numel()
        L.check(L.lib.dwn_stem_forward(C.byref(a), dev.index, _stream(dev)), "dwn_stem_forward")
        ctx.mod = mod; ctx.dtype = dtype; ctx.mode = mode
        ctx.save_for_backward(x, weight, xmom, coef)
        return out

    @staticmethod
    def backward(ctx, dout):
        x, weight, xmom, coef = ctx.saved_tensors
        if ctx.mode == L.BN_EVAL:
            raise RuntimeError(_EVAL_BACKWARD_ERROR)
        bn = ctx.mod.stem[1].bn
        dev = x.device
        B, Cin, T, H, W = x.shape
        C0 = weight.shape[0]
        dout = dout.contiguous()
        dx = None
        if ctx.needs_input_grad[0] and ctx.mode == L.BN_FROZEN:
            dx = torch.empty_like(x)
            g = L.StemInputGradArgs()
            g.dtype = _DT[ctx.dtype]; g.training = ctx.mode; g.B = B; g.Cin = Cin; g.C0 = C0; g.S = T * H * W
            g.w = weight.data_ptr(); g.coef = coef.data_ptr(); g.dout = dout.data_ptr(); g.dx = dx.data_ptr()
            L.check(L.lib.dwn_stem_input_grad(C.byref(g), dev.index, _stream(dev)), "dwn_stem_input_grad")
            if not any(ctx.needs_input_grad[1:4]):
                return dx, None, None, None, None, None, None, None
        dw = grad_out(ctx.mod.stem[0].weight)
        dgamma = grad_out(bn.weight)
        dbeta = grad_out(bn.bias)
        a = L.StemArgs()
        a.dtype = _DT[ctx.dtype]; a.training = ctx.mode; a.B = B; a.Cin = Cin; a.C0 = C0; a.S = T * H * W
        a.eps = bn.eps; a.momentum = bn.momentum
        a.x = x.data_ptr(); a.w = weight.data_ptr(); a.bn = _bn_struct(bn, coef, dgamma, dbeta)
        a.xmom = xmom.data_ptr(); a.dout = dout.data_ptr(); a.dw = dw.data_ptr()
        ws = _ws(L.lib.dwn_stem_workspace_bytes(C.byref(a)), dev)
        a.ws = ws.data_ptr(); a.ws_bytes = ws.numel()
        if ctx.needs_input_grad[0] and ctx.mode == L.BN_TRAIN:
            dx = torch.empty_like(x)
            L.check(L.lib.dwn_stem_backward_input(C.byref(a), dx.data_ptr(), dev.index, _stream(dev)), "dwn_stem_backward_input")
        else:
            L.check(L.lib.dwn_stem_backward(C.byref(a), dev.index, _stream(dev)), "dwn_stem_backward")
        return dx, dw, dgamma, dbeta, None, None, None, None


_BLOCK_PARAMS = ("w_pw", "g1", "b1", "w_dws", "g2", "b2", "w_dwt", "g3", "b3", "se_wr", "se_br", "se_we", "se_be",
                 "w_pwl", "g4", "b4", "gsc", "bsc")


def _block_args(blk, geom, x, dtype, training, coefs, saved, drop_scale, x_has_pe, a0):
    B, T, Hin, Win, Cin = x.shape
    a = L.BlockArgs()
    a.dtype = _DT[dtype]; a.training = int(training)
    a.B = B; a.T = T; a.Hin = Hin; a.Win = Win
    a.Hout = (Hin - 1) // blk.spatial_stride + 1
    a.Wout = (Win - 1) // blk.spatial_stride + 1
    a.Cin = Cin; a.Cmid = blk.mid_features; a.Cout = blk.out_features
    a.stride = blk.spatial_stride; a.ks = blk.spatial_kernel; a.kt = blk.temporal_kernel
    a.se_r = blk.se.conv_reduce.out_channels
    bn1 = blk.conv_pw[1].bn
    a.eps = bn1.eps; a.momentum = bn1.momentum
    a.x = x.data_ptr()
    a.x_has_pe = int(x_has_pe)
    a.a0 = _ptr(a0)
    pe_t, pe_h, pe_w, hsrc, wsrc, hinv, winv = geom
    a.pe_t = pe_t.data_ptr(); a.pe_h = pe_h.data_ptr(); a.pe_w = pe_w.data_ptr()
    a.hsrc = hsrc.data_ptr(); a.wsrc = wsrc.data_ptr(); a.hinv = hinv.data_ptr(); a.winv = winv.data_ptr()
    a.w_pw = blk.conv_pw[0].weight.data_ptr()
    a.w_dws = blk.spat_covn_dw[0].weight.data_ptr()
    a.w_dwt = blk.temp_covn_dw[0].weight.data_ptr()
    a.w_pwl = blk.conv_pwl[0].weight.data_ptr()
    a.se_wr = blk.se.conv_reduce.weight.data_ptr(); a.se_br = blk.se.conv_reduce.bias.data_ptr()
    a.se_we = blk.se.conv_expand.weight.data_ptr(); a.se_be = blk.se.conv_expand.bias.data_ptr()
    a.drop_scale = _ptr(drop_scale)
    a.se_pmean = saved["pmean"].data_ptr(); a.se_hidpre = saved["hidpre"].data_ptr()
    a.se_gate = saved["gate"].data_ptr()
    a.f32_products = _f32_products(blk)
    a.y1_mode = getattr(blk, "_dwn_y1_mode", _Y1_MODE)
    return a


class BlockFn(torch.autograd.Function):

    @staticmethod
    def forward(ctx, x, drop_scale, blk, geom, dtype, x_has_pe, out_pe, mode, *params):
        _require_gpu(x, "BlockFn")
        x = x.contiguous()
        dev = x.device
        B, T, Hin, Win, Cin = x.shape
        s = blk.spatial_stride
        Hout, Wout = (Hin - 1) // s + 1, (Win - 1) // s + 1
        Cmid, Cout = blk.mid_features, blk.out_features
        bns = blk.bn_modules()
        for bn in bns:
            _check_bn(bn)
        training = mode
        f32 = dict(dtype=torch.float32, device=dev)
        y2 = torch.empty(B, T, Hout, Wout, Cmid, dtype=dtype, device=dev)
        z3 = torch.empty_like(y2)
        a0 = None if x_has_pe else torch.empty_like(x)
        y4 = torch.empty(B, T, Hout, Wout, Cout, dtype=dtype, device=dev)
        out = torch.empty_like(y4)
        coefs = [torch.empty(4 * c, **f32) for c in (Cmid, Cmid, Cmid, Cout, Cout)]
        R = blk.se.conv_reduce.out_channels
        saved = dict(pmean=torch.empty(B, Cmid, **f32), hidpre=torch.empty(B, R, **f32),
                     gate=torch.empty(B, Cmid, **f32))
        a = _block_args(blk, geom, x, dtype, training, coefs, saved, drop_scale, x_has_pe, a0)
        a.out = out.data_ptr()
        writes = L.lib.dwn_block_forward_writes(C.byref(a))
        y1 = torch.empty(B, T, Hin, Win, Cmid, dtype=dtype, device=dev) if writes & 1 else None
        y3 = torch.empty_like(y2) if writes & 2 else None
        a.y1 = _ptr(y1); a.y2 = y2.data_ptr(); a.y3 = _ptr(y3); a.y4 = y4.data_ptr()
        a.z3 = z3.data_ptr()
        if out_pe is not None:
            a.out_pe_t, a.out_pe_h, a.out_pe_w = (t.data_ptr() for t in out_pe)
        a.bn1, a.bn2, a.bn3, a.bn4, a.bnsc = (_bn_struct(bn, cf) for bn, cf in zip(bns, coefs))
        ws = _ws(L.lib.dwn_block_workspace_bytes(C.byref(a), 0), dev)
        a.ws = ws.data_ptr(); a.ws_bytes = ws.numel()
        L.check(L.lib.dwn_block_forward(C.byref(a), dev.index, _stream(dev)), "dwn_block_forward")
        ctx.blk = blk; ctx.geom = geom; ctx.dtype = dtype; ctx.mode = mode
        if getattr(blk, "_capture", False):
            blk._captured = dict(y1=y1, y2=y2, y3=y3, y4=y4, z3=z3, coefs=coefs, **saved)
        ctx.has_drop = drop_scale is not None
        if mode == L.BN_EVAL:
            return out
        tensors = [x if x_has_pe else a0, y1, y2, y3, y4, *coefs, saved["pmean"], saved["hidpre"], saved["gate"], z3]
        if drop_scale is not None:
            tensors.append(drop_scale)
        ctx.save_for_backward(*tensors)
        return out

    @staticmethod
    def backward(ctx, dout):
        if ctx.mode == L.BN_EVAL:
            raise RuntimeError(_EVAL_BACKWARD_ERROR)
        blk, dtype = ctx.blk, ctx.dtype
        t = ctx.saved_tensors
        x, y1, y2, y3, y4 = t[:5]
        coefs = list(t[5:10])
        saved = dict(pmean=t[10], hidpre=t[11], gate=t[12])
        z3 = t[13]
        drop_scale = t[14] if ctx.has_drop else None
        dev = x.device
        dout = dout.contiguous()
        B, T, Hin, Win, Cin = x.shape
        Hout, Wout = y2.shape[2], y2.shape[3]
        Cmid, Cout = blk.mid_features, blk.out_features
        f32 = dict(dtype=torch.float32, device=dev)
        a = _block_args(blk, ctx.geom, x, dtype, ctx.mode, coefs, saved, drop_scale, True, None)
        a.y1 = _ptr(y1); a.y2 = y2.data_ptr(); a.y3 = y3.data_ptr(); a.y4 = y4.data_ptr()
        a.z3 = z3.data_ptr()
        bns = blk.bn_modules()
        dg = [grad_out(bn.weight) for bn in bns]
        db = [grad_out(bn.bias) for bn in bns]
        a.bn1, a.bn2, a.bn3, a.bn4, a.bnsc = (_bn_struct(bn, cf, g_, b_) for bn, cf, g_, b_ in zip(bns, coefs, dg, db))
        m_in, m_out = B * T * Hin * Win, B * T * Hout * Wout
        buf_a = torch.empty(max(m_in, m_out) * Cmid, dtype=dtype, device=dev)
        buf_b = torch.empty(m_out * Cmid, dtype=dtype, device=dev)
        dy4 = torch.empty(m_out * Cout, dtype=dtype, device=dev)
        da0 = torch.empty(m_in * Cin, dtype=dtype, device=dev)
        dx = torch.empty_like(x)
        R = blk.se.conv_reduce.out_channels
        dw_pw = grad_out(blk.conv_pw[0].weight)
        dw_dws = grad_out(blk.spat_covn_dw[0].weight)
        dw_dwt = grad_out(blk.temp_covn_dw[0].weight)
        dw_pwl = grad_out(blk.conv_pwl[0].weight)
        dse_wr = grad_out(blk.se.conv_reduce.weight); dse_br = grad_out(blk.se.conv_reduce.bias)
        dse_we = grad_out(blk.se.conv_expand.weight); dse_be = grad_out(blk.se.conv_expand.bias)
        a.dout = dout.data_ptr(); a.dx = dx.data_ptr()
        a.buf_a = buf_a.data_ptr(); a.buf_b = buf_b.data_ptr(); a.dy4 = dy4.data_ptr(); a.da0 = da0.data_ptr()
        a.dw_pw = dw_pw.data_ptr(); a.dw_dws = dw_dws.data_ptr(); a.dw_dwt = dw_dwt.data_ptr()
        a.dw_pwl = dw_pwl.data_ptr()
        a.dse_wr = dse_wr.data_ptr(); a.dse_br = dse_br.data_ptr(); a.dse_we = dse_we.data_ptr()
        a.dse_be = dse_be.data_ptr()
        a.pwl_bwd = _PWL_BWD
        ws = _ws(L.lib.dwn_block_workspace_bytes(C.byref(a), 1), dev)
        a.ws = ws.data_ptr(); a.ws_bytes = ws.numel()
        L.check(L.lib.dwn_block_backward(C.byref(a), dev.index, _stream(dev)), "dwn_block_backward")
        _ddp_flush()
        grads = (dw_pw, dg[0], db[0], dw_dws, dg[1], db[1], dw_dwt, dg[2], db[2], dse_wr, dse_br, dse_we, dse_be,
                 dw_pwl, dg[3], db[3], dg[4], db[4])
        return (dx, None, None, None, None, None, None, None) + grads


class PoolFn(torch.autograd.Function):

    @staticmethod
    def forward(ctx, x):
        _require_gpu(x, "PoolFn")
        x = x.contiguous()
        B, T, H, W, Cc = x.shape
        out = torch.empty(B, T, Cc, dtype=x.dtype, device=x.device)
        a = L.PoolArgs()
        a.dtype = _DT[x.dtype]; a.BT = B * T; a.HW = H * W; a.C = Cc; a.x = x.data_ptr(); a.out = out.data_ptr()
        L.check(L.lib.dwn_pool_forward(C.byref(a), x.device.index, _stream(x.device)), "dwn_pool_forward")
        ctx.shape = (B, T, H, W, Cc)
        return out

    @staticmethod
    def backward(ctx, dout):
        B, T, H, W, Cc = ctx.shape
        dout = dout.contiguous()
        dx = torch.empty(B, T, H, W, Cc, dtype=dout.dtype, device=dout.device)
        a = L.PoolArgs()
        a.dtype = _DT[dout.dtype]; a.BT = B * T; a.HW = H * W; a.C = Cc; a.dout = dout.data_ptr(); a.dx = dx.data_ptr()
        L.check(L.lib.dwn_pool_backward(C.byref(a), dout.device.index, _stream(dout.device)), "dwn_pool_backward")
        return dx


class CortexFn(torch.autograd.Function):

    @staticmethod
    def forward(ctx, x, drop_scale, layer, dtype, mode, weight, g, b, gsc, bsc):
        _require_gpu(x, "CortexFn")
        x = x.contiguous()
        dev = x.device
        B, T, Cin = x.shape
        Cc = layer.out_features
        bn, bnsc = layer.bn.bn, layer.bn_sc.bn
        _check_bn(bn); _check_bn(bnsc)
        y = torch.empty(B, T, Cc, dtype=dtype, device=dev)
        out = torch.empty_like(y)
        coef = torch.empty(4 * Cc, dtype=torch.float32, device=dev)
        coefsc = torch.empty(4 * Cc, dtype=torch.float32, device=dev)
        a = L.CortexArgs()
        a.dtype = _DT[dtype]; a.training = mode; a.B = B; a.T = T; a.Cin = Cin; a.C = Cc
        a.groups = layer.groups; a.eps = bn.eps; a.momentum = bn.momentum
        a.x = x.data_ptr(); a.out = out.data_ptr(); a.y = y.data_ptr(); a.w = weight.data_ptr()
        a.bn = _bn_struct(bn, coef); a.bnsc = _bn_struct(bnsc, coefsc); a.drop_scale = _ptr(drop_scale)
        a.f32_products = _f32_products(layer)
        ws = _ws(L.lib.dwn_cortex_workspace_bytes(C.byref(a), 0), dev)
        a.ws = ws.data_ptr(); a.ws_bytes = ws.numel()
        L.check(L.lib.dwn_cortex_forward(C.byref(a), dev.index, _stream(dev)), "dwn_cortex_forward")
        ctx.layer = layer; ctx.dtype = dtype; ctx.mode = mode; ctx.has_drop = drop_scale is not None
        tensors = [x, y, coef, coefsc, weight]
        if drop_scale is not None:
            tensors.append(drop_scale)
        ctx.save_for_backward(*tensors)
        return out

    @staticmethod
    def backward(ctx, dout):
        if ctx.mode == L.BN_EVAL:
            raise RuntimeError(_EVAL_BACKWARD_ERROR)
        layer, dtype = ctx.layer, ctx.dtype
        t = ctx.saved_tensors
        x, y, coef, coefsc, weight = t[:5]
        drop_scale = t[5] if ctx.has_drop else None
        dev = x.device
        dout = dout.contiguous()
        B, T, Cin = x.shape
        Cc = layer.out_features
        bn, bnsc = layer.bn.bn, layer.bn_sc.bn
        f32 = dict(dtype=torch.float32, device=dev)
        dgm, dbm, dgs, dbs = grad_out(bn.weight), grad_out(bn.bias), grad_out(bnsc.weight), grad_out(bnsc.bias)
        dw = grad_out(layer.conv.weight)
        dx = torch.empty_like(x)
        a = L.CortexArgs()
# ... 802 lines not shown
```

Before: 1477.

## Recompute z3 (BN+SiLU of y3) inside PWL GEMM prologues instead of storing it

For eligible bf16 blocks (Cout 128, large Cmid), the forward SE pool no longer writes the z3 activation. The pointwise-linear forward GEMM and the backward weight-grad GEMM instead recompute BN3 affine plus SiLU from y3 in their A-operand load, with bf16 rounding to match the stored values. A new KD GEMM prologue variant loads the BN scale and shift into LDS alongside the SE gate. This saves a full-size activation write, its read-back and its memory, at the cost of extra ALU work and LDS in the GEMM prologues. The read-only pool kernel uses a deeper unroll.

After: 1485 (median of 6 runs). No clear change (+0.5%).

```diff
diff --git a/include/dwn.h b/include/dwn.h
--- a/include/dwn.h
+++ b/include/dwn.h
@@ -191,6 +191,7 @@
     int pwl_bwd;
     int f32_products;
     int y1_mode;
+    int z3_mode;
 } dwn_block_args;
 
 typedef struct dwn_pool_args {
@@ -308,6 +309,7 @@
 int dwn_block_forward(const dwn_block_args* a, int device, void* stream);
 int dwn_block_backward(const dwn_block_args* a, int device, void* stream);
 int dwn_block_forward_writes(const dwn_block_args* a);
+int dwn_block_stores_z3(const dwn_block_args* a);
 int dwn_pool_forward(const dwn_pool_args* a, int device, void* stream);
 int dwn_pool_backward(const dwn_pool_args* a, int device, void* stream);
 size_t dwn_cortex_workspace_bytes(const dwn_cortex_args* a, int backward);
diff --git a/sensorium_amd/_lib.py b/sensorium_amd/_lib.py
--- a/sensorium_amd/_lib.py
+++ b/sensorium_amd/_lib.py
@@ -113,7 +113,7 @@
                 ("dout", c_p), ("dx", c_p), ("buf_a", c_p), ("buf_b", c_p), ("dy4", c_p), ("da0", c_p),
                 ("dw_pw", c_p), ("dw_dws", c_p), ("dw_dwt", c_p), ("dw_pwl", c_p), ("dse_wr", c_p),
                 ("dse_br", c_p), ("dse_we", c_p), ("dse_be", c_p),
-                ("ws", c_p), ("ws_bytes", c_sz), ("pwl_bwd", c_i), ("f32_products", c_i), ("y1_mode", c_i)]
+                ("ws", c_p), ("ws_bytes", c_sz), ("pwl_bwd", c_i), ("f32_products", c_i), ("y1_mode", c_i), ("z3_mode", c_i)]
 
 
 class PoolArgs(C.Structure):
@@ -319,6 +319,7 @@
     "dwn_block_forward": (c_i, [_P(BlockArgs), c_i, c_p]),
     "dwn_block_backward": (c_i, [_P(BlockArgs), c_i, c_p]),
     "dwn_block_forward_writes": (c_i, [_P(BlockArgs)]),
+    "dwn_block_stores_z3": (c_i, [_P(BlockArgs)]),
     "dwn_pool_forward": (c_i, [_P(PoolArgs), c_i, c_p]),
     "dwn_pool_backward": (c_i, [_P(PoolArgs), c_i, c_p]),
     "dwn_cortex_workspace_bytes": (c_sz, [_P(CortexArgs), c_i]),
@@ -421,7 +422,7 @@
                            "dwn_trial_score_finalize", "dwn_spatial_gain_ws_bytes", "dwn_spatial_gain_forward",
                            "dwn_spatial_gain_backward", "dwn_noise_forward", "dwn_sta_state_bytes", "dwn_sta_ws_bytes",
                            "dwn_sta_accumulate", "dwn_sta_finalize", "dwn_gauss2d_ws_bytes", "dwn_gauss2d_fit",
-                           "dwn_gauss2d_profile") and not hasattr(lib, name):
+                           "dwn_gauss2d_profile", "dwn_block_stores_z3") and not hasattr(lib, name):
             continue
         fn = getattr(lib, name)
         fn.restype = restype
diff --git a/sensorium_amd/csrc/dwn_api.hip b/sensorium_amd/csrc/dwn_api.hip
--- a/sensorium_amd/csrc/dwn_api.hip
+++ b/sensorium_amd/csrc/dwn_api.hip
@@ -198,6 +198,13 @@
     d.dy.ld = a.Cmid; d.y1.ld = a.Cmid; d.a0_ld = a.Cin; d.Cin = a.Cin;
     if (!dw_spatial_bwd_rc_supported(d, a.dtype)) return false;
     return a.y1_mode == 2 || a.Cin == 64;
+}
+static bool block_z3_free(const dwn_block_args& a) {
+    if (a.training != DWN_BN_TRAIN || a.z3_mode == 1 || !pwl_bwd_per_sample(a)) return false;
+    if (a.z3_mode == 2) return true;
+    const i64 S = (i64)a.T * a.Hout * a.Wout;
+    return a.dtype == DWN_BF16 && !pwl_gated_weights(a) && a.Cout == 128 && S % 128 == 0 && a.Cmid % 128 == 0 && a.Cmid >= 512 &&
+           a.Cmid <= 4096 && (i64)a.B * S >= 8192;
 }
 static bool block_fwd_rc(const dwn_block_args& a) {
     return !a.training && dwn_dw_spatial_rc_supported(a.dtype, a.Cin, a.Cmid, a.ks, a.stride, a.Hin, a.Win) != 0;
@@ -580,23 +587,27 @@
         PROF(DWN_FAM_DWT_FWD, launch_dw_temporal_fwd(d, dt, s));
     }
     if (bs) TRY(bn_finalize(w.st3, a.Cmid, (double)Mout, a.bn3, a.Cmid, 1, a.momentum, a.eps, s));
+    const bool z3_free = block_z3_free(a);
     if (!eval_z3) {
+        if (!z3_free && !a.z3) return dwn_set_error(-1, "block_forward: z3 buffer required (dwn_block_stores_z3)");
         LoadDesc z3 = ld_bnact(a.y3, a.Cmid, a.bn3.coef, a.Cmid, 1, nullptr, 0, S_out);
-        PROF(DWN_FAM_SE_POOL, k_se_pool(z3, a.B, a.Cmid, S_out, w.pooled, a.z3, dt, s));
+        PROF(DWN_FAM_SE_POOL, k_se_pool(z3, a.B, a.Cmid, S_out, w.pooled, z3_free ? nullptr : a.z3, dt, s));
     }
     int gate_folded = 0;
     TRY(k_se_mlp_fwd(w.pooled, 1.0f / (float)S_out, a.se_wr, a.se_br, a.se_we, a.se_be, a.B, a.Cmid, a.se_r,
                      a.se_pmean, a.se_hidpre, a.se_gate, pwl_gated_weights(a) ? a.w_pwl : nullptr, w.wgated, a.Cout, dt, &gate_folded, s));
     if (pwl_gated_weights(a)) {
         if (!gate_folded) TRY(k_gate_weights(a.w_pwl, a.se_gate, w.wgated, a.B, a.Cout, a.Cmid, dt, s));
-        GemmNN g = nn_base(ld_plain(a.z3, a.Cmid), LD_PLAIN, w.wgated, a.Cmid, a.y4, a.Cout, (int)Mout, a.Cout, a.Cmid, 1);
+        const LoadDesc u = z3_free ? ld_bnact(a.y3, a.Cmid, a.bn3.coef, a.Cmid, 1, nullptr, 0, S_out) : ld_plain(a.z3, a.Cmid);
+        GemmNN g = nn_base(u, z3_free ? LD_BNACT : LD_PLAIN, w.wgated, a.Cmid, a.y4, a.Cout, (int)Mout, a.Cout, a.Cmid, 1);
         g.b_sample_stride = (i64)a.Cout * a.Cmid; g.b_rows_per_sample = S_out;
         g.stats = tr ? w.st4 : nullptr; g.stat_nchan = a.Cout; g.f32_split = f32_split_of(a.f32_products, !tr);
         PROF(DWN_FAM_PWL_FWD, launch_gemm_nn(g, dt, s));
     } else {
         LoadDesc u = ld_plain(a.z3, a.Cmid);
         u.gate = a.se_gate; u.gate_ld = a.Cmid; u.rows_per_sample = S_out;
-        GemmNN g = nn_base(u, LD_GATE, w.wpwl, a.Cmid, a.y4, a.Cout, (int)Mout, a.Cout, a.Cmid, 1);
+        if (z3_free) u = ld_bnact(a.y3, a.Cmid, a.bn3.coef, a.Cmid, 2, a.se_gate, a.Cmid, S_out);
+        GemmNN g = nn_base(u, z3_free ? LD_BNACT : LD_GATE, w.wpwl, a.Cmid, a.y4, a.Cout, (int)Mout, a.Cout, a.Cmid, 1);
         g.stats = tr ? w.st4 : nullptr; g.stat_nchan = a.Cout; g.f32_split = f32_split_of(a.f32_products, !tr);
         PROF(DWN_FAM_PWL_FWD, launch_gemm_nn(g, dt, s));
     }
@@ -685,7 +696,10 @@
     void* du = a.buf_a;
     if (w.pb) {
         {
-            GemmTN g = tn_base(ld_plain(a.dy4, a.Cout), LD_PLAIN, ld_plain(a.z3, a.Cmid), LD_PLAIN, (int)Mout, a.Cout,
+            const bool z3_free = block_z3_free(a);
+            if (!z3_free && !a.z3) return dwn_set_error(-1, "block_backward: z3 buffer required (dwn_block_stores_z3)");
+            const LoadDesc q = z3_free ? ld_bnact(a.y3, a.Cmid, a.bn3.coef, a.Cmid, 1, nullptr, 0, S_out) : ld_plain(a.z3, a.Cmid);
+            GemmTN g = tn_base(ld_plain(a.dy4, a.Cout), LD_PLAIN, q, z3_free ? LD_BNACT : LD_PLAIN, (int)Mout, a.Cout,
                                a.Cmid, w.pb, a.Cmid, 1);
             g.rows_per_sample = S_out; g.dw_sample_stride = (i64)a.Cout * a.Cmid;
             PROF(DWN_FAM_PWL_WGRAD, launch_gemm_tn(g, dt, s));
@@ -763,6 +777,7 @@
     }
     return 1;
 }
+int dwn_block_stores_z3(const dwn_block_args* ap) { return block_z3_free(*ap) ? 0 : 1; }
 
 int dwn_pool_forward(const dwn_pool_args* a, int device, void* stream) {
     ENTER(device);
diff --git a/sensorium_amd/csrc/dwn_common.h b/sensorium_amd/csrc/dwn_common.h
--- a/sensorium_amd/csrc/dwn_common.h
+++ b/sensorium_amd/csrc/dwn_common.h
@@ -200,6 +200,10 @@
 #pragma unroll
         for (int i = 0; i < KC; ++i) o[i] = fmaf(o[i], s[i], t[i]);
         if (d.act) silu_n<KC>(o);
+        if (d.act == 2) {
+#pragma unroll
+            for (int i = 0; i < KC; ++i) o[i] = round_t<T>(o[i]);
+        }
         if (d.gate) {
             int b = (int)(r32 / (unsigned)d.rows_per_sample);
             float g[KC];
@@ -277,6 +281,10 @@
 #pragma unroll
             for (int i = 0; i < KC; ++i) o[i] = fmaf(o[i], c1[i], c2[i]);
             if (d.act) silu_n<KC>(o);
+            if (d.act == 2) {
+                const uint4 z = pack16<T>(o);
+                unpack16<T>(z, o);
+            }
             if (d.gate) {
                 gate_for(d, row);
 #pragma unroll
diff --git a/sensorium_amd/csrc/dwn_elementwise.hip b/sensorium_amd/csrc/dwn_elementwise.hip
--- a/sensorium_amd/csrc/dwn_elementwise.hip
+++ b/sensorium_amd/csrc/dwn_elementwise.hip
@@ -1120,7 +1120,7 @@
     return 0;
 }
 
-template <typename T>
+template <typename T, int U>
 __global__ __launch_bounds__(256) void se_pool_kernel(LoadDesc z3, int C, int rows_per_sample, int chunks,
                                                       long long* pooled, T* z3out) {
     SLICE_SETUP(C)
@@ -1139,15 +1139,15 @@
         ld_coef<KC>(z3.v1 + chan, sc);
         ld_coef<KC>(z3.v2 + chan, sh);
         const T* yp = reinterpret_cast<const T*>(z3.p);
-        for (int r0 = r_beg + pl; r0 < r_end; r0 += 4 * 32) {
-            uint4 raw[4];
-#pragma unroll
-            for (int u = 0; u < 4; ++u) {
+        for (int r0 = r_beg + pl; r0 < r_end; r0 += U * 32) {
+            uint4 raw[U];
+#pragma unroll
+            for (int u = 0; u < U; ++u) {
                 int r = r0 + 32 * u;
                 raw[u] = *reinterpret_cast<const uint4*>(yp + ((i64)b * rows_per_sample + (r < r_end ? r : r_beg)) * z3.ld + chan);
             }
 #pragma unroll
-            for (int u = 0; u < 4; ++u) {
+            for (int u = 0; u < U; ++u) {
                 int r = r0 + 32 * u;
                 if (r >= r_end) break;
                 float v[KC];
@@ -1176,9 +1176,16 @@
     if (chunks > maxchunks) chunks = maxchunks;
     if (chunks < 1) chunks = 1;
     dim3 grid(B * chunks, slices);
+    if (!z3out) {
+        DISPATCH_T(dtype,
+            hipLaunchKernelGGL((se_pool_kernel<bf16_t, 8>), grid, dim3(256), 0, s, z3, C, rows_per_sample, chunks, pooled, (bf16_t*)nullptr),
+            hipLaunchKernelGGL((se_pool_kernel<float, 8>), grid, dim3(256), 0, s, z3, C, rows_per_sample, chunks, pooled, (float*)nullptr));
+        DWN_CHECK_LAUNCH();
+        return 0;
+    }
     DISPATCH_T(dtype,
-        hipLaunchKernelGGL((se_pool_kernel<bf16_t>), grid, dim3(256), 0, s, z3, C, rows_per_sample, chunks, pooled, (bf16_t*)z3out),
-        hipLaunchKernelGGL((se_pool_kernel<float>), grid, dim3(256), 0, s, z3, C, rows_per_sample, chunks, pooled, (float*)z3out));
+        hipLaunchKernelGGL((se_pool_kernel<bf16_t, 4>), grid, dim3(256), 0, s, z3, C, rows_per_sample, chunks, pooled, (bf16_t*)z3out),
+        hipLaunchKernelGGL((se_pool_kernel<float, 4>), grid, dim3(256), 0, s, z3, C, rows_per_sample, chunks, pooled, (float*)z3out));
     DWN_CHECK_LAUNCH();
     return 0;
 }
diff --git a/sensorium_amd/csrc/dwn_gemm_kd.hip b/sensorium_amd/csrc/dwn_gemm_kd.hip
--- a/sensorium_amd/csrc/dwn_gemm_kd.hip
+++ b/sensorium_amd/csrc/dwn_gemm_kd.hip
@@ -25,6 +25,7 @@
     int M, N, K;
     const float* bias;
     const float* gate; int gate_ld, rows_per_sample;
+    const float* bn_s; const float* bn_t; int act;
     double* stats; int stat_nchan;
     int ntm, ntn;
 };
@@ -35,7 +36,7 @@
     asm volatile("" ::: "memory");
 }
 
-template <int BN, int RT, bool GATE, bool CAT>
+template <int BN, int RT, int PRO, bool CAT>
 __global__ __launch_bounds__(256, BN * RT >= 512 ? 2 : KD_MINW128) void gemm_kd_kernel(const KdArgs g) {
     constexpr int BM = 64 * RT;
     constexpr int NJ = BN / 16;
@@ -108,9 +109,15 @@
     for (int u = 0; u < 4; ++u) load_a(u, ar[u]);
     load_b(0, bs[0]);
     load_b(1, bs[1]);
-    if constexpr (GATE) {
+    if constexpr (PRO != 0) {
         const float* grow = g.gate + (i64)(m0 / g.rows_per_sample) * g.gate_ld;
-        for (int k = tid * 4; k < g.K; k += 1024) *reinterpret_cast<float4*>(sgate + k) = *reinterpret_cast<const float4*>(grow + k);
+        for (int k = tid * 4; k < g.K; k += 1024) {
+            *reinterpret_cast<float4*>(sgate + k) = *reinterpret_cast<const float4*>(grow + k);
+            if constexpr (PRO == 2) {
+                *reinterpret_cast<float4*>(sgate + g.K + k) = *reinterpret_cast<const float4*>(g.bn_s + k);
+                *reinterpret_cast<float4*>(sgate + 2 * g.K + k) = *reinterpret_cast<const float4*>(g.bn_t + k);
+            }
+        }
     }
     store_b(0, bs[0]);
     load_b(2, bs[0]);
@@ -131,7 +138,7 @@
             uint4 af[RT];
 #pragma unroll
             for (int i = 0; i < RT; ++i) af[i] = ar[u][i];
-            if constexpr (GATE) {
+            if constexpr (PRO == 1) {
                 const float4 g0 = *reinterpret_cast<const float4*>(sgate + (ks << 5) + 8 * lg);
                 const float4 g1 = *reinterpret_cast<const float4*>(sgate + (ks << 5) + 8 * lg + 4);
                 const float gv[8] = {g0.x, g0.y, g0.z, g0.w, g1.x, g1.y, g1.z, g1.w};
@@ -142,6 +149,31 @@
 #pragma unroll
                     for (int e = 0; e < 8; ++e) v[e] *= gv[e];
                     af[i] = pack16<bf16_t>(v);
+                }
+            }
+            if constexpr (PRO == 2) {
+                const float* const cg = sgate + (ks << 5) + 8 * lg;
+#pragma unroll
+                for (int h = 0; h < 2; ++h) {
+                    const float4 g4 = *reinterpret_cast<const float4*>(cg + 4 * h);
+                    const float4 s4 = *reinterpret_cast<const float4*>(cg + g.K + 4 * h);
+                    const float4 t4 = *reinterpret_cast<const float4*>(cg + 2 * g.K + 4 * h);
+#pragma unroll
+                    for (int i = 0; i < RT; ++i) {
+                        const uint32_t w0 = h ? af[i].z : af[i].x, w1 = h ? af[i].w : af[i].y;
+                        float v[4] = {__uint_as_float(w0 << 16), __uint_as_float(w0 & 0xffff0000u),
+                                      __uint_as_float(w1 << 16), __uint_as_float(w1 & 0xffff0000u)};
+                        v[0] = fmaf(v[0], s4.x, t4.x); v[1] = fmaf(v[1], s4.y, t4.y);
+                        v[2] = fmaf(v[2], s4.z, t4.z); v[3] = fmaf(v[3], s4.w, t4.w);
+                        if (g.act) silu_n<4>(v);
+                        if (g.act == 2) {
+                            const uint32_t z0 = pk_bf16(v[0], v[1]), z1 = pk_bf16(v[2], v[3]);
+                            v[0] = __uint_as_float(z0 << 16); v[1] = __uint_as_float(z0 & 0xffff0000u);
+                            v[2] = __uint_as_float(z1 << 16); v[3] = __uint_as_float(z1 & 0xffff0000u);
+                        }
+                        const uint32_t o0 = pk_bf16(v[0] * g4.x, v[1] * g4.y), o1 = pk_bf16(v[2] * g4.z, v[3] * g4.w);
+                        if (h) { af[i].z = o0; af[i].w = o1; } else { af[i].x = o0; af[i].y = o1; }
+                    }
                 }
             }
             const unsigned char* const st = fb + (u & 1) * STG;
@@ -227,14 +259,16 @@
 static bool kd_args_ok(const GemmNN& g, int dtype) {
     if (dtype != DWN_BF16 || g.groups != 1 || g.b_sample_stride || g.M < 1) return false;
     if (g.epi == EPI_STORE) {
-        if (g.a_kind != LD_PLAIN && g.a_kind != LD_GATE) return false;
+        if (g.a_kind != LD_PLAIN && g.a_kind != LD_GATE && g.a_kind != LD_BNACT) return false;
         if (g.a2) return false;
     } else if (g.epi == EPI_STORE_CAT) {
         if (g.a_kind != LD_PLAIN || !g.a2 || !g.bias || g.K1 <= 0 || g.K1 % 32 || g.a2_ld % 8 || ((size_t)g.a2 & 15) || ((size_t)g.bias & 15)) return false;
     } else {
         return false;
     }
-    if (g.a_kind == LD_GATE && (!g.a.gate || g.a.rows_per_sample <= 0 || g.a.rows_per_sample % 128 || g.a.gate_ld % 4 || ((size_t)g.a.gate & 15) || g.K > 4096))
+    if (g.a_kind == LD_BNACT && (!g.a.gate || !g.a.v1 || !g.a.v2 || (((size_t)g.a.v1 | (size_t)g.a.v2) & 15) || g.a.act < 0 || g.a.act > 2))
+        return false;
+    if ((g.a_kind == LD_GATE || g.a_kind == LD_BNACT) && (!g.a.gate || g.a.rows_per_sample <= 0 || g.a.rows_per_sample % 128 || g.a.gate_ld % 4 || ((size_t)g.a.gate & 15) || g.K > 4096))
         return false;
     if (g.K % 128 || g.N % 128 || g.a.ld % 8 || g.ldb % 8 || g.ldc % 8) return false;
     if (((size_t)g.a.p | (size_t)g.b | (size_t)g.c) & 15) return false;
@@ -245,19 +279,19 @@
     if (g.variant == DWN_NN_TILE128 || g.variant == DWN_NN_XL128 || g.variant == DWN_NN_XL256) return false;
     if (!kd_args_ok(g, dtype)) return false;
     if (g.variant == DWN_NN_KD) return true;
-    return g.K >= 512 && g.M >= 8192 && (g.N == 256 || (g.N == 128 && g.a_kind == LD_GATE));
-}
-
-template <int BN, int RT, bool GATE, bool CAT>
+    return g.K >= 512 && g.M >= 8192 && (g.N == 256 || (g.N == 128 && (g.a_kind == LD_GATE || g.a_kind == LD_BNACT)));
+}
+
+template <int BN, int RT, int PRO, bool CAT>
 static int launch_kd_t(const KdArgs& a, hipStream_t s) {
-    const size_t smem = 2 * (size_t)BN * 64 + 64 * ((size_t)BN * 2 + 16) + 2 * (size_t)BN * 4 + (GATE ? (size_t)a.K * 4 : 0);
+    const size_t smem = 2 * (size_t)BN * 64 + 64 * ((size_t)BN * 2 + 16) + 2 * (size_t)BN * 4 + (PRO == 2 ? 3 : PRO) * (size_t)a.K * 4;
     {
-        hipError_t e = lds_opt_in(gemm_kd_kernel<BN, RT, GATE, CAT>, smem);
+        hipError_t e = lds_opt_in(gemm_kd_kernel<BN, RT, PRO, CAT>, smem);
         if (e != hipSuccess) return dwn_set_error((int)e, hipGetErrorString(e));
     }
     const unsigned tiles = (unsigned)a.ntm * (unsigned)a.ntn;
     const unsigned grid = (tiles + 7u) & ~7u;
-    hipLaunchKernelGGL((gemm_kd_kernel<BN, RT, GATE, CAT>), dim3(grid), dim3(256), smem, s, a);
+    hipLaunchKernelGGL((gemm_kd_kernel<BN, RT, PRO, CAT>), dim3(grid), dim3(256), smem, s, a);
     DWN_CHECK_LAUNCH();
     return 0;
 }
@@ -271,17 +305,20 @@
     a.C = reinterpret_cast<bf16_t*>(g.c); a.ldc = g.ldc;
     a.M = g.M; a.N = g.N; a.K = g.K;
     a.bias = cat ? g.bias : nullptr;
-    const bool gate = g.a_kind == LD_GATE;
+    const bool bnact = g.a_kind == LD_BNACT;
+    const bool gate = g.a_kind == LD_GATE || bnact;
+    a.bn_s = bnact ? g.a.v1 : nullptr; a.bn_t = bnact ? g.a.v2 : nullptr; a.act = bnact ? g.a.act : 0;
     a.gate = gate ? g.a.gate : nullptr; a.gate_ld = gate ? g.a.gate_ld : 0; a.rows_per_sample = gate ? g.a.rows_per_sample : 1;
     a.stats = g.stats; a.stat_nchan = g.stat_nchan;
     const int ntm128 = (g.M + 127) / 128;
-    const bool wide = KD_WIDE && g.N % 256 == 0 && (i64)ntm128 * (g.N / 256) >= 512;
+    const bool wide = KD_WIDE && !bnact && g.N % 256 == 0 && (i64)ntm128 * (g.N / 256) >= 512;
     a.ntm = ntm128;
     a.ntn = wide ? g.N / 256 : g.N / 128;
     if (wide) {
-        if (gate) return launch_kd_t<256, 2, true, false>(a, s);
-        return cat ? launch_kd_t<256, 2, false, true>(a, s) : launch_kd_t<256, 2, false, false>(a, s);
-    }
-    if (gate) return launch_kd_t<128, 2, true, false>(a, s);
-    return cat ? launch_kd_t<128, 2, false, true>(a, s) : launch_kd_t<128, 2, false, false>(a, s);
-}
+        if (gate) return launch_kd_t<256, 2, 1, false>(a, s);
+        return cat ? launch_kd_t<256, 2, 0, true>(a, s) : launch_kd_t<256, 2, 0, false>(a, s);
+    }
+    if (bnact) return launch_kd_t<128, 2, 2, false>(a, s);
+    if (gate) return launch_kd_t<128, 2, 1, false>(a, s);
+    return cat ? launch_kd_t<128, 2, 0, true>(a, s) : launch_kd_t<128, 2, 0, false>(a, s);
+}
diff --git a/sensorium_amd/csrc/dwn_gemm_tn.hip b/sensorium_amd/csrc/dwn_gemm_tn.hip
--- a/sensorium_amd/csrc/dwn_gemm_tn.hip
+++ b/sensorium_amd/csrc/dwn_gemm_tn.hip
@@ -12,7 +12,7 @@
 template <> struct TnCfg<float>  { static constexpr int PAD = 64; };
 
 template <int PLD, int QLD> struct TnOcc {
-    static constexpr int value = (PLD == LD_AFFINE2 || PLD == LD_DY3 || QLD == LD_AFFINE2 || QLD == LD_DY3) ? 2 : TN_MINW_PLAIN;
+    static constexpr int value = (PLD == LD_AFFINE2 || PLD == LD_DY3 || QLD == LD_AFFINE2 || QLD == LD_DY3 || QLD == LD_BNACT) ? 2 : TN_MINW_PLAIN;
 };
 template <typename T, int PLD, int QLD>
 __global__ __launch_bounds__(256, (TnOcc<PLD, QLD>::value)) void gemm_tn_kernel(const GemmTN g) {
diff --git a/sensorium_amd/ops.py b/sensorium_amd/ops.py
--- a/sensorium_amd/ops.py
+++ b/sensorium_amd/ops.py
@@ -109,6 +109,7 @@
 
 _PWL_BWD = _env_choice("DWN_PWL_BWD", {"": 0, "new": 1, "old": 2})
 _Y1_MODE = _env_choice("DWN_Y1", {"": 0, "free": 0, "materialise": 1, "all": 2})
+_Z3_MODE = _env_choice("DWN_Z3", {"": 0, "store": 1, "free": 2})
 
 
 def grad_out(param: torch.Tensor, zero: bool = False) -> torch.Tensor:
@@ -256,7 +257,14 @@
     a.se_gate = saved["gate"].data_ptr()
     a.f32_products = _f32_products(blk)
     a.y1_mode = getattr(blk, "_dwn_y1_mode", _Y1_MODE)
+    a.z3_mode = getattr(blk, "_dwn_z3_mode", _Z3_MODE)
+    a.pwl_bwd = _PWL_BWD
     return a
+
+
+def _stores_z3(a) -> bool:
+    fn = getattr(L.lib, "dwn_block_stores_z3", None)
+    return True if fn is None else bool(fn(C.byref(a)))
 
 
 class BlockFn(torch.autograd.Function):
@@ -276,7 +284,6 @@
         training = mode
         f32 = dict(dtype=torch.float32, device=dev)
         y2 = torch.empty(B, T, Hout, Wout, Cmid, dtype=dtype, device=dev)
-        z3 = torch.empty_like(y2)
         a0 = None if x_has_pe else torch.empty_like(x)
         y4 = torch.empty(B, T, Hout, Wout, Cout, dtype=dtype, device=dev)
         out = torch.empty_like(y4)
@@ -290,7 +297,8 @@
         y1 = torch.empty(B, T, Hin, Win, Cmid, dtype=dtype, device=dev) if writes & 1 else None
         y3 = torch.empty_like(y2) if writes & 2 else None
         a.y1 = _ptr(y1); a.y2 = y2.data_ptr(); a.y3 = _ptr(y3); a.y4 = y4.data_ptr()
-        a.z3 = z3.data_ptr()
+        z3 = torch.empty_like(y2) if _stores_z3(a) else None
+        a.z3 = _ptr(z3)
         if out_pe is not None:
             a.out_pe_t, a.out_pe_h, a.out_pe_w = (t.data_ptr() for t in out_pe)
         a.bn1, a.bn2, a.bn3, a.bn4, a.bnsc = (_bn_struct(bn, cf) for bn, cf in zip(bns, coefs))
@@ -328,7 +336,7 @@
         f32 = dict(dtype=torch.float32, device=dev)
         a = _block_args(blk, ctx.geom, x, dtype, ctx.mode, coefs, saved, drop_scale, True, None)
         a.y1 = _ptr(y1); a.y2 = y2.data_ptr(); a.y3 = y3.data_ptr(); a.y4 = y4.data_ptr()
-        a.z3 = z3.data_ptr()
+        a.z3 = _ptr(z3)
         bns = blk.bn_modules()
         dg = [grad_out(bn.weight) for bn in bns]
         db = [grad_out(bn.bias) for bn in bns]
@@ -352,7 +360,6 @@
         a.dw_pwl = dw_pwl.data_ptr()
         a.dse_wr = dse_wr.data_ptr(); a.dse_br = dse_br.data_ptr(); a.dse_we = dse_we.data_ptr()
         a.dse_be = dse_be.data_ptr()
-        a.pwl_bwd = _PWL_BWD
         ws = _ws(L.lib.dwn_block_workspace_bytes(C.byref(a), 1), dev)
         a.ws = ws.data_ptr(); a.ws_bytes = ws.numel()
         L.check(L.lib.dwn_block_backward(C.byref(a), dev.index, _stream(dev)), "dwn_block_backward")
```
